# harryjfowen/PointsToWood

Measured on AMD Instinct MI355X. Metric: classified points/sec, higher is better.
Workload: dtype f16x3

## Files before the change

### include/p2w.h

```cpp
#ifndef P2W_H
#define P2W_H

#include <stddef.h>
#include <stdint.h>

#ifdef __cplusplus
extern "C" {
#endif

typedef void* p2w_stream_t;

#define P2W_OK 0
#define P2W_EINVAL (-1)
#define P2W_ENULL (-2)
#define P2W_EALIGN (-3)
#define P2W_EWORKSPACE (-4)
#define P2W_EUNSUPPORTED (-5)

#define P2W_MAX_K 64
#define P2W_MAX_K_WIDE 100
#define P2W_MAX_K_CONV 32

int32_t p2w_version(void);
const char* p2w_strerror(int32_t code);
// ... 36 lines not shown

#define P2W_SEARCH_X_INDEX_IN_W 1
#define P2W_SEARCH_Q_ROW_IN_W 2
#define P2W_SEARCH_BOX 4

int32_t p2w_ball_query(const float* xyzr_x, const int32_t* ptr_x, const float* xyzr_q, const int32_t* qidx,
                       const int32_t* ptr_q, int32_t B, int32_t m_bound, double r, int32_t cap, int32_t* nbr,
                       int32_t* deg, const float* tile_bbox, int32_t flags, p2w_stream_t stream);

int32_t p2w_knn(const float* xyzr_x, const int32_t* ptr_x, const float* xyzr_q, const int32_t* qidx,
                const int32_t* ptr_q, int32_t B, int32_t m_bound, int32_t k, int32_t* nbr, int32_t* deg,
                const float* tile_bbox, int32_t flags, p2w_stream_t stream);

int32_t p2w_knn_grid(const float* xyzr_x, const uint64_t* keys_x, const int32_t* ptr_x, const p2w_grid* grid,
                     const float* xyzr_q, const int32_t* qidx, const int32_t* ptr_q, int32_t B, int32_t m_bound,
                     int32_t k, int32_t* nbr, int32_t* deg, const float* hint, int32_t flags, p2w_stream_t stream);
int32_t p2w_knn_hint2(const float* xyzr_q, const int32_t* rank, const int32_t* ptr_q, int32_t B, int32_t m_bound,
                      const float* xyzr_c, float* hint, p2w_stream_t stream);
int32_t p2w_ball_query_grid(const float* xyzr_x, const uint64_t* keys_x, const int32_t* ptr_x, const p2w_grid* grid,
                            const float* xyzr_q, const int32_t* qidx, const int32_t* ptr_q, int32_t B, int32_t m_bound,
                            double r, int32_t cap, int32_t* nbr, int32_t* deg, int32_t flags, p2w_stream_t stream);
int32_t p2w_voxel_sample_table_prepare(void* ws, size_t ws_bytes, p2w_stream_t stream);
int32_t p2w_voxel_sample_table_prepared(const float* xyzr, const int32_t* ptr, int32_t B, int32_t n_bound, float res,
                                        int32_t* idx_out, int32_t* ptr_out, int32_t* batch_out, int32_t* order_out,
                                        uint64_t* sorted_keys_out, uint64_t* cell_keys_out, p2w_grid* grid_out, int32_t* inv_out,
                                        int32_t* rank_sorted_out, int32_t* cell_start_out, int32_t* cell_start_sorted_out,
                                        int32_t* status_out, int64_t table_cells, void* ws, size_t ws_bytes, p2w_stream_t stream);

int32_t p2w_knn_grid_indexed(const float* xyzr_x, const uint64_t* keys_x, const int32_t* ptr_x, const p2w_grid* grid,
                             const int32_t* cell_start, const float* xyzr_q, const int32_t* qidx, const int32_t* ptr_q, int32_t B,
                             int32_t m_bound, int32_t k, int32_t* nbr, int32_t* deg, const float* hint, int32_t flags,
                             p2w_stream_t stream);
int32_t p2w_ball_query_grid_indexed(const float* xyzr_x, const uint64_t* keys_x, const int32_t* ptr_x, const p2w_grid* grid,
                                    const int32_t* cell_start, const float* xyzr_q, const int32_t* qidx, const int32_t* ptr_q,
                                    int32_t B, int32_t m_bound, double r, int32_t cap, int32_t* nbr, int32_t* deg, int32_t flags,
                                    p2w_stream_t stream);


size_t p2w_morton_order_ws_bytes(int32_t n);
int32_t p2w_morton_order(const float* xyzr, int32_t n, const p2w_grid* grid, int32_t* order_out, void* ws, size_t ws_bytes,
                         p2w_stream_t stream);

#define P2W_CELL_NONFINITE INT64_MAX
int32_t p2w_cells_nd(const float* P, int32_t n, int32_t D, int32_t ld, float size, int64_t* cell_out, void* ws, size_t ws_bytes,
                     p2w_stream_t stream);
size_t p2w_sort_pairs_u64_ws_bytes(int32_t n);
int32_t p2w_sort_pairs_u64(const uint64_t* keys_in, uint64_t* keys_out, const int32_t* vals_in, int32_t* vals_out, int32_t n, void* ws,
                           size_t ws_bytes, p2w_stream_t stream);
size_t p2w_key_runs_ws_bytes(int32_t n);
int32_t p2w_key_runs(const uint64_t* keys_sorted, int32_t n, int32_t min_count, int32_t* starts_out, int32_t* counts_out, int32_t* n_out,
                     void* ws, size_t ws_bytes, p2w_stream_t stream);

size_t p2w_cell_starts_ws_bytes(int64_t n_cells);
int32_t p2w_cell_starts(const uint64_t* keys_sorted, int32_t n, int64_t n_cells, int32_t* table_out, void* ws, size_t ws_bytes,
                        p2w_stream_t stream);

int32_t p2w_knn_refine_f64(const double* cand_sorted, const int32_t* cand_index, const int32_t* cand_pos,
                           const uint64_t* keys_sorted, const int32_t* cell_start, const p2w_grid* grid, double ox, double oy,
                           double oz, const double* q, int32_t m, int32_t nc, int32_t k, int32_t* nbr, int32_t* deg,
                           p2w_stream_t stream);

#define P2W_CLUSTER_LINK 1
#define P2W_CLUSTER_COMPRESS 2
#define P2W_CLUSTER_NUMBER 4
#define P2W_CLUSTER_ALL 7
size_t p2w_euclid_cluster_ws_bytes(int64_t n);
int32_t p2w_euclid_cluster(const double* xyz_sorted, const int32_t* order, const uint64_t* keys_sorted, const int32_t* cell_start,
                           const p2w_grid* grid, int64_t n, double tolerance, int64_t min_size, int64_t max_size, int32_t stages,
                           int64_t* labels_out, int32_t* counts_out, uint64_t* pairs_out, void* ws, size_t ws_bytes,
                           p2w_stream_t stream);

int32_t p2w_knn_wide_f64(const double* xyz_sorted, const int32_t* order, const uint64_t* keys_sorted, const int32_t* cell_start,
                         const p2w_grid* grid, int64_t n, int32_t k, double slack, int32_t* nbr_out, p2w_stream_t stream);

size_t p2w_pathlen_grow_ws_bytes(int64_t n);
int32_t p2w_pathlen_grow(const double* xyz, const int32_t* nbr, int64_t n, int32_t k, int32_t base, int32_t kpairs, double nbrs_threshold,
                         double nbrs_threshold_step, double graph_threshold, int32_t* step_out, int32_t* edges_out, int64_t edge_cap,
                         int64_t* info_out, double* threshold_out, void* ws, size_t ws_bytes, p2w_stream_t stream);

size_t p2w_pathlen_sssp_ws_bytes(int64_t n, int64_t n_edges);
int32_t p2w_pathlen_sssp(const double* xyz, const int32_t* edges, int64_t n_edges, int64_t n, int32_t base, double* dist_out,
                         int32_t* parent_out, int64_t* info_out, void* ws, size_t ws_bytes, p2w_stream_t stream);

int32_t p2w_pathlen_weights(const double* xyz, const int64_t* edges, int64_t n_edges, double* w_out, p2w_stream_t stream);

#define P2W_EVAL_CHUNK 4096
#define P2W_EVAL_MAX_CLASSES 8
size_t p2w_confusion_ws_bytes(int64_t n, int32_t segments, int32_t classes);
int32_t p2w_confusion(const float* truth, const float* pred, const double* weight, const int64_t* seg_ptr, int64_t n, int32_t segments,
                      int32_t classes, int64_t* counts, double* wsum, int64_t* invalid, void* ws, size_t ws_bytes,
                      p2w_stream_t stream);

#define P2W_LOSS_CHUNK 4096
size_t p2w_poly1_focal_ws_bytes(int64_t n);
int32_t p2w_poly1_focal(const float* logits, const float* labels, const float* weight, int64_t weight_n, int64_t n, double epsilon,
                        double gamma, double alpha, double label_smoothing, double eps, float* loss, float* dloss, double* sum,
                        void* ws, size_t ws_bytes, p2w_stream_t stream);

int32_t p2w_vote(const int32_t* nbr, const int32_t* deg, int32_t k, const float* pred, const float* prob, int32_t n,
                 float any_wood, float* label_out, float* pwood_out, p2w_stream_t stream);

int32_t p2w_tile_bbox(const float* xyzr, const int32_t* ptr, int32_t B, int32_t n_bound, float* bbox, p2w_stream_t stream);
int32_t p2w_tile_bbox_count(int32_t B, int32_t n_bound);


int32_t p2w_stem(const float* xyzr, int32_t n, const float* w, const float* b, int32_t C, float* out,
                 p2w_stream_t stream);

typedef struct p2w_epilogue {
    const float* bias;
    const float* sc0;
    const float* sh0;
    const float* sc1;
    const float* sh1;
    const float* residual;
    int32_t ldr;
    int32_t relu0, relu1, relu2, relu_final;
    uint32_t* range;
    const void* interp;
    int32_t interp_rows;
} p2w_epilogue;

#define P2W_RANGE_HI 6.0e4f
#define P2W_RANGE_LO 0.03125f
#define P2W_RANGE_SLOTS 16
#define P2W_RANGE_WORDS (64 * P2W_RANGE_SLOTS)

void p2w_packed_dims(int32_t N, int32_t K, int32_t* N_pad, int32_t* K_pad);

int32_t p2w_gemm(const float* A, int32_t lda, const float* Wp, int32_t M, int32_t N, int32_t K,
                 const p2w_epilogue* epi, float* out, int32_t ldo, p2w_stream_t stream);

int32_t p2w_sa_conv(const float* P, int32_t ldp, const float* xyzr_src, const int32_t* idx, const int32_t* batch_dst,
                    const float* sf, const int32_t* nbr, const int32_t* deg, int32_t kw, int32_t M,
                    const float* w1r4 , const float* W2p, int32_t C1, int32_t C2,
                    const float* b2, const float* bn_s, const float* bn_t, float* out, int32_t ldo,
                    p2w_stream_t stream);

#define P2W_PREC_F16X3 0
#define P2W_PREC_F16 1
#define P2W_PREC_BF16 2
int32_t p2w_packed_dims_h(int32_t prec, int32_t N, int32_t K, int32_t* N_pad, int32_t* K_pad);

#define P2W_GEMM_TILE_128 1
#define P2W_GEMM_TILE_256 2
#define P2W_GEMM_GENERIC_EPI 4
#define P2W_GEMM_ORDER_ROWS 8
#define P2W_GEMM_ORDER_COLS 16
#define P2W_GEMM_RESIDUAL_H 32
#define P2W_GEMM_STREAMK 64
#define P2W_GEMM_NO_STREAMK 128
#define P2W_GEMM_TILE_64 (1 << 24)
#define P2W_GEMM_NO_TILE_64 (1 << 25)
#define P2W_SA_ITEM_256 1
#define P2W_SA_ITEM_128 2
#define P2W_SA_PACK8 4

int32_t p2w_gemm_h2(int32_t prec, const void* A_h, int32_t ldh_a, const void* Wh, float wscale, int32_t M, int32_t N,
                    int32_t K, const p2w_epilogue* epi, float* out_f32, int32_t ldo, void* out_h, int32_t ldh_o,
                    int32_t flags, p2w_stream_t stream);
size_t p2w_gemm_h2_sk_ws_bytes(void);
int32_t p2w_gemm_h2_sk(int32_t prec, const void* A_h, int32_t ldh_a, const void* Wh, float wscale, int32_t M, int32_t N,
                       int32_t K, const p2w_epilogue* epi, float* out_f32, int32_t ldo, void* out_h, int32_t ldh_o,
                       void* ws, size_t ws_bytes, int32_t flags, p2w_stream_t stream);
size_t p2w_gemm_h2_rowdot_ws_bytes(int32_t M, int32_t N);
int32_t p2w_gemm_h2_rowdot(int32_t prec, const void* A_h, int32_t ldh_a, const void* Wh, float wscale, int32_t M, int32_t N,
                           int32_t K, const p2w_epilogue* epi, const float* dot_w, float dot_b, float* out, void* ws,
                           size_t ws_bytes, int32_t flags, p2w_stream_t stream);
size_t p2w_sa_conv_h_ws_bytes(int32_t M, int32_t flags);
int32_t p2w_sa_conv_h(int32_t prec, const float* P, int32_t ldp, int32_t n_src, const float* xyzr_src, const int32_t* idx,
                      const int32_t* batch_dst, const float* sf, const int32_t* nbr, const int32_t* deg, int32_t kw,
                      int32_t M, const float* w1r4, const void* W2h, float wscale, int32_t C1, int32_t C2,
                      const float* b2, const float* bn_s, const float* bn_t, float* out, int32_t ldo, void* out_h,
                      int32_t ldh, void* ws, size_t ws_bytes, int32_t flags, p2w_stream_t stream);
int32_t p2w_sa_conv_h_rows(int32_t prec, const float* P, int32_t ldp, int32_t n_src, const float* xyzr_src, const int32_t* idx,
                           const int32_t* batch_dst, const float* sf, const int32_t* nbr, const int32_t* deg, int32_t kw,
                           int32_t M, const float* w1r4, const void* W2h, float wscale, int32_t C1, int32_t C2,
                           const float* b2, const float* bn_s, const float* bn_t, float* out, int32_t ldo, void* out_h,
                           int32_t ldh, void* ws, size_t ws_bytes, int32_t flags, const int32_t* src_row, uint32_t* range,
                           p2w_stream_t stream);
int32_t p2w_stem_h2(int32_t prec, const float* xyzr, int32_t n, const float* w, const float* b, int32_t C, float* out,
                    void* out_h, int32_t ldh, uint32_t* range, p2w_stream_t stream);
int32_t p2w_stem_h2_indexed(int32_t prec, const float* xyzr, int32_t n, const float* w, const float* b, int32_t C, float* out,
                            void* out_h, int32_t ldh, uint32_t* range, p2w_stream_t stream);
int32_t p2w_interp_concat_h2(int32_t prec, const float* xc, int32_t Fc, const float* xyzr_c, const float* xyzr_f,
                             const int32_t* nbr, const int32_t* deg, int32_t kw, const float* skip, int32_t Fs, int32_t m,
                             void* out_h, int32_t ldh, p2w_stream_t stream);
int32_t p2w_interp_weights(const float* xyzr_c, const float* xyzr_f, const int32_t* nbr, const int32_t* deg, int32_t kw, int32_t m,
                           void* records, p2w_stream_t stream);
int32_t p2w_concat_xyz_h2(int32_t prec, const float* x, int32_t F, const float* xyzr, int32_t m, void* out_h, int32_t ldh,
                          p2w_stream_t stream);

int32_t p2w_interp_concat(const float* xc, int32_t Fc, const float* xyzr_c, const float* xyzr_f, const int32_t* nbr,
                          const int32_t* deg, int32_t kw, const float* skip, int32_t Fs, int32_t m, float* out,
                          int32_t ldo, p2w_stream_t stream);

int32_t p2w_concat_xyz(const float* x, int32_t F, const float* xyzr, int32_t m, float* out, int32_t ldo,
                       p2w_stream_t stream);

int32_t p2w_segment_max(const float* x, int32_t ldx, int32_t F, const int32_t* ptr, int32_t B, float* out,
                        p2w_stream_t stream);

int32_t p2w_rowdot(const float* x, int32_t ldx, int32_t F, const float* w, float b, int32_t m, float* out,
                   p2w_stream_t stream);

int32_t p2w_fill_batch_nbr(const int32_t* batch, int32_t m, int32_t* nbr, int32_t* deg, p2w_stream_t stream);


int32_t p2w_segment_max_arg(const float* x, int32_t ldx, int32_t F, const int32_t* ptr, int32_t B, float* out, int32_t* arg,
                            p2w_stream_t stream);
int32_t p2w_segment_max_bwd(const float* grad_out, int32_t ldg, const int32_t* arg, const int32_t* ptr, int32_t B, int32_t F,
                            float* grad_x, int32_t ldx, int32_t n, p2w_stream_t stream);
size_t p2w_interp_bwd_ws_bytes(int32_t m, int32_t kw, int32_t n_coarse);
int32_t p2w_interp_bwd(const float* grad_out, int32_t ldg, int32_t F, const float* xyzr_c, const float* xyzr_f, const int32_t* nbr,
                       const int32_t* deg, int32_t kw, int32_t m, int32_t n_coarse, float* grad_x, int32_t ldx, void* ws,
                       size_t ws_bytes, p2w_stream_t stream);

int32_t p2w_edge_l1(const float* P, int32_t ldp, const float* rec_src, const float* rec_dst, const int32_t* ptr, const int32_t* src,
                    const float* Wg, int32_t n_src, int32_t M, int32_t E, int32_t C1, float* geo, float* H1, int32_t ldh,
                    p2w_stream_t stream);
#define P2W_EDGE_CHUNK 1024
size_t p2w_edge_l1_bwd_ws_bytes(int32_t E, int32_t n_src, int32_t C1);
int32_t p2w_edge_l1_bwd(const float* gH, int32_t ldg, const float* H1, int32_t ldh, const float* geo, const int32_t* src,
                        const float* Wg, int32_t n_src, int32_t E, int32_t C1, float* gP, int32_t ldgp, float* gR, float* gWg, void* ws,
                        size_t ws_bytes, p2w_stream_t stream);

#define P2W_BN_GROUP 16
size_t p2w_relu_bn_max_ws_bytes(int32_t E, int32_t M, int32_t C2);
int32_t p2w_relu_bn_max(const float* z, int32_t ldz, const int32_t* ptr, const float* gamma, const float* beta, float* running_mean,
                        float* running_var, double momentum, double eps, int32_t E, int32_t M, int32_t C2, float* out, float* ext,
                        int32_t* arg, float* mean, float* invstd, void* ws, size_t ws_bytes, p2w_stream_t stream);
int32_t p2w_relu_bn_max_bwd(const float* g, const float* z, int32_t ldz, const int32_t* ptr, const int32_t* arg, const float* ext,
                            const float* mean, const float* invstd, const float* gamma, int32_t E, int32_t M, int32_t C2, float* dz,
                            int32_t lddz, float* dgamma, float* dbeta, void* ws, size_t ws_bytes, p2w_stream_t stream);

#ifdef __cplusplus
}
#endif
#endif
```

### pointstowood_amd/_lib.py

```python
from __future__ import annotations

import ctypes as C
import os

import torch

_HERE = os.path.dirname(os.path.abspath(__file__))
LIB_PATH = os.path.join(_HERE, "libp2w_gfx950.so")

_vp, _i32, _f32, _sz = C.c_void_p, C.c_int32, C.c_float, C.c_size_t


class Epilogue(C.Structure):
    _fields_ = [("bias", _vp), ("sc0", _vp), ("sh0", _vp), ("sc1", _vp), ("sh1", _vp), ("residual", _vp),
                ("ldr", _i32), ("relu0", _i32), ("relu1", _i32), ("relu2", _i32), ("relu_final", _i32), ("range", _vp),
                ("interp", _vp), ("interp_rows", _i32)]


SEARCH_X_INDEX_IN_W, SEARCH_Q_ROW_IN_W, SEARCH_BOX = 1, 2, 4
PREC_F16X3, PREC_F16, PREC_BF16 = 0, 1, 2
PREC_OF = {"f16x3": PREC_F16X3, "fp16": PREC_F16, "bf16": PREC_BF16}
GEMM_TILE_128, GEMM_TILE_256, GEMM_GENERIC_EPI, GEMM_ORDER_ROWS, GEMM_ORDER_COLS, GEMM_RESIDUAL_H = 1, 2, 4, 8, 16, 32
GEMM_STREAMK, GEMM_NO_STREAMK = 64, 128
SA_ITEM_256, SA_ITEM_128, SA_PACK8 = 1, 2, 4
CLUSTER_LINK, CLUSTER_COMPRESS, CLUSTER_NUMBER, CLUSTER_ALL = 1, 2, 4, 7
MAX_K_WIDE = 100
EVAL_CHUNK, EVAL_MAX_CLASSES = 4096, 8
LOSS_CHUNK = 4096
EDGE_CHUNK = 1024
BN_GROUP = 16

SIGNATURES = {
    "p2w_version": (_i32, []),
    "p2w_strerror": (C.c_char_p, [_i32]),
    "p2w_pack_xyzr": (_i32, [_vp, _i32, _vp, _vp, _i32, _i32, _vp, _vp, _vp]),
    "p2w_voxel_sample_ws_bytes": (_sz, [_i32]),
    "p2w_voxel_sample": (_i32, [_vp, _vp, _i32, _i32, _f32, _vp, _vp, _vp, _vp, _vp, _vp, _vp, _vp, _vp, _vp, _sz, _vp]),
    "p2w_voxel_sample_table_ws_bytes": (_sz, [_i32, C.c_int64]),
    "p2w_voxel_sample_table": (_i32, [_vp, _vp, _i32, _i32, _f32, _vp, _vp, _vp, _vp, _vp, _vp, _vp, _vp, _vp, _vp, _vp, _vp, C.c_int64,
                                      _vp, _sz, _vp]),
    "p2w_voxel_sample_table_prepare": (_i32, [_vp, _sz, _vp]),
    "p2w_voxel_sample_table_prepared": (_i32, [_vp, _vp, _i32, _i32, _f32, _vp, _vp, _vp, _vp, _vp, _vp, _vp, _vp, _vp, _vp, _vp, _vp, C.c_int64,
                                               _vp, _sz, _vp]),
    "p2w_knn_grid_indexed": (_i32, [_vp, _vp, _vp, _vp, _vp, _vp, _vp, _vp, _i32, _i32, _i32, _vp, _vp, _vp, _i32, _vp]),
    "p2w_ball_query_grid_indexed": (_i32, [_vp, _vp, _vp, _vp, _vp, _vp, _vp, _vp, _i32, _i32, C.c_double, _i32, _vp, _vp, _i32, _vp]),
    "p2w_knn_hint2": (_i32, [_vp, _vp, _vp, _i32, _i32, _vp, _vp, _vp]),
    "p2w_knn_grid": (_i32, [_vp, _vp, _vp, _vp, _vp, _vp, _vp, _i32, _i32, _i32, _vp, _vp, _vp, _i32, _vp]),
    "p2w_ball_query_grid": (_i32, [_vp, _vp, _vp, _vp, _vp, _vp, _vp, _i32, _i32, C.c_double, _i32, _vp, _vp, _i32, _vp]),
    "p2w_index_records": (_i32, [_vp, _vp, _vp, _i32, _i32, _vp, _vp]),
    "p2w_voxel_grid": (_i32, [_vp, _vp, _i32, _i32, _f32, _vp, _vp, _sz, _vp]),
    "p2w_consecutive_cluster": (_i32, [_vp, _i32, _vp, _vp, _vp, _vp, _sz, _vp]),
    "p2w_level_gather": (_i32, [_vp, _vp, _vp, _vp, _i32, _i32, _vp, _vp, _vp]),
    "p2w_ball_query": (_i32, [_vp, _vp, _vp, _vp, _vp, _i32, _i32, C.c_double, _i32, _vp, _vp, _vp, _i32, _vp]),
    "p2w_knn": (_i32, [_vp, _vp, _vp, _vp, _vp, _i32, _i32, _i32, _vp, _vp, _vp, _i32, _vp]),
    "p2w_morton_order_ws_bytes": (_sz, [_i32]),
    "p2w_morton_order": (_i32, [_vp, _i32, _vp, _vp, _vp, _sz, _vp]),
    "p2w_cells_nd": (_i32, [_vp, _i32, _i32, _i32, _f32, _vp, _vp, _sz, _vp]),
    "p2w_sort_pairs_u64_ws_bytes": (_sz, [_i32]),
    "p2w_sort_pairs_u64": (_i32, [_vp, _vp, _vp, _vp, _i32, _vp, _sz, _vp]),
    "p2w_key_runs_ws_bytes": (_sz, [_i32]),
    "p2w_key_runs": (_i32, [_vp, _i32, _i32, _vp, _vp, _vp, _vp, _sz, _vp]),
    "p2w_knn_refine_f64": (_i32, [_vp, _vp, _vp, _vp, _vp, _vp, C.c_double, C.c_double, C.c_double, _vp, _i32, _i32, _i32, _vp, _vp, _vp]),
    "p2w_cell_starts_ws_bytes": (_sz, [C.c_int64]),
    "p2w_cell_starts": (_i32, [_vp, _i32, C.c_int64, _vp, _vp, _sz, _vp]),
    "p2w_vote": (_i32, [_vp, _vp, _i32, _vp, _vp, _i32, _f32, _vp, _vp, _vp]),
    "p2w_euclid_cluster_ws_bytes": (_sz, [C.c_int64]),
    "p2w_euclid_cluster": (_i32, [_vp, _vp, _vp, _vp, _vp, C.c_int64, C.c_double, C.c_int64, C.c_int64, _i32, _vp, _vp, _vp, _vp, _sz, _vp]),
    "p2w_knn_wide_f64": (_i32, [_vp, _vp, _vp, _vp, _vp, C.c_int64, _i32, C.c_double, _vp, _vp]),
    "p2w_pathlen_grow_ws_bytes": (_sz, [C.c_int64]),
    "p2w_pathlen_grow": (_i32, [_vp, _vp, C.c_int64, _i32, _i32, _i32, C.c_double, C.c_double, C.c_double, _vp, _vp, C.c_int64, _vp, _vp,
                                _vp, _sz, _vp]),
    "p2w_pathlen_sssp_ws_bytes": (_sz, [C.c_int64, C.c_int64]),
    "p2w_pathlen_sssp": (_i32, [_vp, _vp, C.c_int64, C.c_int64, _i32, _vp, _vp, _vp, _vp, _sz, _vp]),
    "p2w_pathlen_weights": (_i32, [_vp, _vp, C.c_int64, _vp, _vp]),
    "p2w_confusion_ws_bytes": (_sz, [C.c_int64, _i32, _i32]),
    "p2w_confusion": (_i32, [_vp, _vp, _vp, _vp, C.c_int64, _i32, _i32, _vp, _vp, _vp, _vp, _sz, _vp]),
    "p2w_poly1_focal_ws_bytes": (_sz, [C.c_int64]),
    "p2w_poly1_focal": (_i32, [_vp, _vp, _vp, C.c_int64, C.c_int64, C.c_double, C.c_double, C.c_double, C.c_double, C.c_double, _vp, _vp, _vp,
                               _vp, _sz, _vp]),
    "p2w_tile_bbox": (_i32, [_vp, _vp, _i32, _i32, _vp, _vp]),
    "p2w_tile_bbox_count": (_i32, [_i32, _i32]),
    "p2w_stem": (_i32, [_vp, _i32, _vp, _vp, _i32, _vp, _vp]),
    "p2w_packed_dims": (None, [_i32, _i32, C.POINTER(_i32), C.POINTER(_i32)]),
    "p2w_gemm": (_i32, [_vp, _i32, _vp, _i32, _i32, _i32, C.POINTER(Epilogue), _vp, _i32, _vp]),
    "p2w_sa_conv": (_i32, [_vp, _i32, _vp, _vp, _vp, _vp, _vp, _vp, _i32, _i32, _vp, _vp, _i32, _i32, _vp, _vp, _vp,
                           _vp, _i32, _vp]),
    "p2w_packed_dims_h": (_i32, [_i32, _i32, _i32, C.POINTER(_i32), C.POINTER(_i32)]),
    "p2w_gemm_h2": (_i32, [_i32, _vp, _i32, _vp, _f32, _i32, _i32, _i32, C.POINTER(Epilogue), _vp, _i32, _vp, _i32, _i32, _vp]),
    "p2w_gemm_h2_sk_ws_bytes": (_sz, []),
    "p2w_gemm_h2_sk": (_i32, [_i32, _vp, _i32, _vp, _f32, _i32, _i32, _i32, C.POINTER(Epilogue), _vp, _i32, _vp, _i32, _vp, _sz, _i32, _vp]),
    "p2w_gemm_h2_rowdot_ws_bytes": (_sz, [_i32, _i32]),
    "p2w_gemm_h2_rowdot": (_i32, [_i32, _vp, _i32, _vp, _f32, _i32, _i32, _i32, C.POINTER(Epilogue), _vp, _f32, _vp, _vp, _sz, _i32, _vp]),
    "p2w_sa_conv_h_ws_bytes": (_sz, [_i32, _i32]),
    "p2w_sa_conv_h": (_i32, [_i32, _vp, _i32, _i32, _vp, _vp, _vp, _vp, _vp, _vp, _i32, _i32, _vp, _vp, _f32, _i32, _i32, _vp, _vp,
                             _vp, _vp, _i32, _vp, _i32, _vp, _sz, _i32, _vp]),
    "p2w_stem_h2": (_i32, [_i32, _vp, _i32, _vp, _vp, _i32, _vp, _vp, _i32, _vp, _vp]),
    "p2w_stem_h2_indexed": (_i32, [_i32, _vp, _i32, _vp, _vp, _i32, _vp, _vp, _i32, _vp, _vp]),
    "p2w_sa_conv_h_rows": (_i32, [_i32, _vp, _i32, _i32, _vp, _vp, _vp, _vp, _vp, _vp, _i32, _i32, _vp, _vp, _f32, _i32, _i32, _vp, _vp,
                                  _vp, _vp, _i32, _vp, _i32, _vp, _sz, _i32, _vp, _vp, _vp]),
    "p2w_interp_concat_h2": (_i32, [_i32, _vp, _i32, _vp, _vp, _vp, _vp, _i32, _vp, _i32, _i32, _vp, _i32, _vp]),
    "p2w_interp_weights": (_i32, [_vp, _vp, _vp, _vp, _i32, _i32, _vp, _vp]),
    "p2w_concat_xyz_h2": (_i32, [_i32, _vp, _i32, _vp, _i32, _vp, _i32, _vp]),
    "p2w_interp_concat": (_i32, [_vp, _i32, _vp, _vp, _vp, _vp, _i32, _vp, _i32, _i32, _vp, _i32, _vp]),
    "p2w_concat_xyz": (_i32, [_vp, _i32, _vp, _i32, _vp, _i32, _vp]),
    "p2w_segment_max": (_i32, [_vp, _i32, _i32, _vp, _i32, _vp, _vp]),
    "p2w_rowdot": (_i32, [_vp, _i32, _i32, _vp, _f32, _i32, _vp, _vp]),
    "p2w_fill_batch_nbr": (_i32, [_vp, _i32, _vp, _vp, _vp]),
    "p2w_segment_max_arg": (_i32, [_vp, _i32, _i32, _vp, _i32, _vp, _vp, _vp]),
    "p2w_segment_max_bwd": (_i32, [_vp, _i32, _vp, _vp, _i32, _i32, _vp, _i32, _i32, _vp]),
    "p2w_interp_bwd_ws_bytes": (_sz, [_i32, _i32, _i32]),
    "p2w_interp_bwd": (_i32, [_vp, _i32, _i32, _vp, _vp, _vp, _vp, _i32, _i32, _i32, _vp, _i32, _vp, _sz, _vp]),
    "p2w_edge_l1": (_i32, [_vp, _i32, _vp, _vp, _vp, _vp, _vp, _i32, _i32, _i32, _i32, _vp, _vp, _i32, _vp]),
    "p2w_edge_l1_bwd_ws_bytes": (_sz, [_i32, _i32, _i32]),
    "p2w_edge_l1_bwd": (_i32, [_vp, _i32, _vp, _i32, _vp, _vp, _vp, _i32, _i32, _i32, _vp, _i32, _vp, _vp, _vp, _sz, _vp]),
    "p2w_relu_bn_max_ws_bytes": (_sz, [_i32, _i32, _i32]),
    "p2w_relu_bn_max": (_i32, [_vp, _i32, _vp, _vp, _vp, _vp, _vp, C.c_double, C.c_double, _i32, _i32, _i32, _vp, _vp, _vp, _vp, _vp, _vp, _sz,
                               _vp]),
    "p2w_relu_bn_max_bwd": (_i32, [_vp, _vp, _i32, _vp, _vp, _vp, _vp, _vp, _vp, _i32, _i32, _i32, _vp, _i32, _vp, _vp, _vp, _sz, _vp]),
}

_lib = None


def lib():
    global _lib
    if _lib is None:
        from . import build as _build
        if _build._stale():
            try:
                _build.build()
            except Exception as e:
                raise RuntimeError(
                    f"{LIB_PATH} is missing or stale and could not be rebuilt ({e}). The HIP extension is the "
                    "only compute path (no CPU fallback). Build it with `python -m pointstowood_amd.build`.") from e
        h = C.CDLL(LIB_PATH)
        for name, (res, args) in SIGNATURES.items():
            fn = getattr(h, name)
            fn.restype, fn.argtypes = res, args
        _lib = h
    return _lib


def check(code: int, what: str = "") -> None:
    if code != 0:
        msg = lib().p2w_strerror(code).decode()
        raise RuntimeError(f"{what or 'p2w'} failed: {msg} (code {code})")


def ptr(t):
    return None if t is None else t.data_ptr()


_raw_stream = getattr(torch._C, "_cuda_getCurrentRawStream", None)
_raw_device = getattr(torch._C, "_cuda_getDevice", None)


def stream():
    if _raw_stream is not None and _raw_device is not None:
        return _raw_stream(_raw_device())
    return torch.cuda.current_stream().cuda_stream


def stage_timer(on: bool):
    events = []

    def mark():
        if on:
            events.append(torch.cuda.Event(enable_timing=True))
            events[-1].record()

    def ms():
        events[-1].synchronize()
        return [a.elapsed_time(b) for a, b in zip(events[:-1], events[1:])]
    return mark, ms


def require_cuda(*tensors):
    for t in tensors:
        if t is not None and not t.is_cuda:
            raise RuntimeError("pointstowood_amd operators need tensors on an MI355X (cuda) device; "
                               "there is no CPU fallback")


def aligned16(t):
    return t.clone() if t.data_ptr() % 16 else t


def packed_dims(n: int, k: int, prec: int | None = None):
    a, b = _i32(), _i32()
    if prec is None:
        lib().p2w_packed_dims(n, k, C.byref(a), C.byref(b))
    else:
        check(lib().p2w_packed_dims_h(prec, n, k, C.byref(a), C.byref(b)), "p2w_packed_dims_h")
    return a.value, b.value
```

### pointstowood_amd/csrc/p2w_feat.hip

```cpp
#include "p2w_hgemm.h"

constexpr int G_BM = 128, G_BN = 128, G_BK = 32, G_LD = 36;

extern "C" void p2w_packed_dims(int32_t N, int32_t K, int32_t* N_pad, int32_t* K_pad) {
    if (N_pad) *N_pad = (N + 255) / 256 * 256;
    if (K_pad) *K_pad = (K + G_BK - 1) / G_BK * G_BK;
}
extern "C" int32_t p2w_packed_dims_h(int32_t prec, int32_t N, int32_t K, int32_t* N_pad, int32_t* K_pad) {
    if (prec < P2W_PREC_F16X3 || prec > P2W_PREC_BF16) return P2W_EINVAL;
    const int ka = prec == P2W_PREC_F16X3 ? 32 : 64;
    if (N_pad) *N_pad = (N + 255) / 256 * 256;
    if (K_pad) *K_pad = (K + ka - 1) / ka * ka;
    return P2W_OK;
}

__device__ __forceinline__ void mma_slab(const float* __restrict__ As, const float* __restrict__ Bs, int wr, int wc, int lane,
                                         f32x16 (&acc)[2][2]) {
    const int r = lane & 31, h = lane >> 5;
#pragma unroll
    for (int kk = 0; kk < G_BK; kk += 8) {
        const float4 a0 = *reinterpret_cast<const float4*>(&As[(wr * 64 + r) * G_LD + kk + 4 * h]);
        const float4 a1 = *reinterpret_cast<const float4*>(&As[(wr * 64 + 32 + r) * G_LD + kk + 4 * h]);
        const float4 b0 = *reinterpret_cast<const float4*>(&Bs[(wc * 64 + r) * G_LD + kk + 4 * h]);
        const float4 b1 = *reinterpret_cast<const float4*>(&Bs[(wc * 64 + 32 + r) * G_LD + kk + 4 * h]);
// ... 129 lines not shown
    const int h = lane >> 5;
#pragma unroll
    for (int i = 0; i < 2; ++i) {
        const int tgt = t0 + wr * 2 + i;
        if (tgt >= M) continue;
        const int d = min(deg[tgt], kw);
#pragma unroll
        for (int j = 0; j < 2; ++j) {
            const int col = n0 + wc * 64 + j * 32 + (lane & 31);
            const bool cv = col < C2;
            const float bias = cv ? b2[col] : 0.f, s = cv ? bn_s[col] : 0.f, t = cv ? bn_t[col] : 0.f;
            float vmax = -INFINITY;
#pragma unroll
            for (int r = 0; r < 16; ++r) {
                const int slot = (r & 3) + 8 * (r >> 2) + 4 * h;
                const float v = fmaf(fmaxf(fmaf(acc[i][j][r], wscale, bias), 0.f), s, t);
                if (slot < d) vmax = fmaxf(vmax, v);
            }
            vmax = fmaxf(vmax, __shfl_xor(vmax, 32));
            if (d == 0) vmax = 0.f;
            if (cv && h == 0) out[(size_t)tgt * ldo + col] = vmax;
        }
    }
}

__device__ __forceinline__ void sa_row_geometry(int tid, int t0, int M, int kw, const float4* __restrict__ xyzr,
                                                const int* __restrict__ idx, const int* __restrict__ batch_dst,
                                                const float* __restrict__ sf, const int* __restrict__ nbr,
                                                const int* __restrict__ deg, int* m_j, float (*m_g)[4]) {
    if (tid < G_BM) {
        const int tgt = t0 + (tid >> 5), slot = tid & 31;
        int j = 0;
        float rx = 0.f, ry = 0.f, rz = 0.f, rf = 0.f, nrm = 0.f;
        if (tgt < M) {
            const int d = deg[tgt];
            const float s = sf[batch_dst[tgt]];
            const float4 pi = xyzr[idx[tgt]];
            const bool valid = slot < d && slot < kw;
            j = nbr[(size_t)tgt * kw + (valid ? slot : 0)];
            if (j < 0) j = idx[tgt];
            const float4 pj = xyzr[j];
            if (valid) {
                rx = pj.x / s - pi.x / s; ry = pj.y / s - pi.y / s; rz = pj.z / s - pi.z / s;
                nrm = sqrtf(((rx * rx) + (ry * ry)) + (rz * rz));
                rf = pj.w;
            }
        }
        float dmax = nrm;
#pragma unroll
        for (int off = 16; off >= 1; off >>= 1) dmax = fmaxf(dmax, __shfl_xor(dmax, off));
        const float den = dmax + 1e-8f;
        m_j[tid] = j;
        m_g[tid][0] = rx / den; m_g[tid][1] = ry / den; m_g[tid][2] = rz / den; m_g[tid][3] = rf;
    }
}

__device__ __forceinline__ void sa_load_h1(const float* __restrict__ P, int ldp, const float* __restrict__ w1r4, int C1,
                                           int C1pad, int k, const int (&rj)[4], const float4 (&rg)[4], float4 (&ra)[4]) {
    if (k < C1) {
        const float4 wx = *reinterpret_cast<const float4*>(&w1r4[0 * C1pad + k]);
        const float4 wy = *reinterpret_cast<const float4*>(&w1r4[1 * C1pad + k]);
        const float4 wz = *reinterpret_cast<const float4*>(&w1r4[2 * C1pad + k]);
        const float4 wf = *reinterpret_cast<const float4*>(&w1r4[3 * C1pad + k]);
#pragma unroll
        for (int i = 0; i < 4; ++i) {
            const float4 p = *reinterpret_cast<const float4*>(&P[(size_t)rj[i] * ldp + k]);
            const float4 g = rg[i];
            float4 v;
            v.x = fmaxf(fmaf(g.w, wf.x, fmaf(g.z, wz.x, fmaf(g.y, wy.x, fmaf(g.x, wx.x, p.x)))), 0.f);
            v.y = fmaxf(fmaf(g.w, wf.y, fmaf(g.z, wz.y, fmaf(g.y, wy.y, fmaf(g.x, wx.y, p.y)))), 0.f);
            v.z = fmaxf(fmaf(g.w, wf.z, fmaf(g.z, wz.z, fmaf(g.y, wy.z, fmaf(g.x, wx.z, p.z)))), 0.f);
            v.w = fmaxf(fmaf(g.w, wf.w, fmaf(g.z, wz.w, fmaf(g.y, wy.w, fmaf(g.x, wx.w, p.w)))), 0.f);
            ra[i] = v;
        }
    } else {
#pragma unroll
        for (int i = 0; i < 4; ++i) ra[i] = make_float4(0.f, 0.f, 0.f, 0.f);
    }
}

__global__ __launch_bounds__(256) void sa_conv_kernel(const float* __restrict__ P, int ldp, const float4* __restrict__ xyzr,
                                                      const int* __restrict__ idx, const int* __restrict__ batch_dst,
                                                      const float* __restrict__ sf, const int* __restrict__ nbr,
                                                      const int* __restrict__ deg, int kw, int M,
                                                      const float* __restrict__ w1r4, int C1, int C1pad,
                                                      const float* __restrict__ W2p, int C2, int nMt, int nNt,
                                                      const float* __restrict__ b2, const float* __restrict__ bn_s,
                                                      const float* __restrict__ bn_t, float* __restrict__ out, int ldo) {
    __shared__ __attribute__((aligned(16))) float As[G_BM * G_LD];
    __shared__ __attribute__((aligned(16))) float Bs[G_BN * G_LD];
    __shared__ int m_j[G_BM];
    __shared__ float m_g[G_BM][4];
    int mt, nt;
    if (!tile_coords(nMt, nNt, &mt, &nt)) return;
    const int t0 = mt * 4, n0 = nt * G_BN;
    const int tid = threadIdx.x, lane = tid & 63, wave = tid >> 6, wr = wave >> 1, wc = wave & 1;
    const int lrow = tid >> 3, lkq = tid & 7;

    sa_row_geometry(tid, t0, M, kw, xyzr, idx, batch_dst, sf, nbr, deg, m_j, m_g);
    __syncthreads();
    int rj[4];
    float4 rg[4];
#pragma unroll
    for (int i = 0; i < 4; ++i) {
        rj[i] = m_j[lrow + 32 * i];
        rg[i] = *reinterpret_cast<const float4*>(&m_g[lrow + 32 * i][0]);
    }

    f32x16 acc[2][2];
#pragma unroll
    for (int i = 0; i < 2; ++i)
#pragma unroll
        for (int j = 0; j < 2; ++j)
#pragma unroll
            for (int r = 0; r < 16; ++r) acc[i][j][r] = 0.f;

    float4 ra[4], rb[4];
    sa_load_h1(P, ldp, w1r4, C1, C1pad, 4 * lkq, rj, rg, ra);
    load_w_tile(W2p, C1pad, n0, 0, lrow, lkq, rb);
    for (int k0 = 0; k0 < C1pad; k0 += G_BK) {
        __syncthreads();
        store_tile(As, lrow, lkq, ra);
        store_tile(Bs, lrow, lkq, rb);
        __syncthreads();
        if (k0 + G_BK < C1pad) {
            sa_load_h1(P, ldp, w1r4, C1, C1pad, k0 + G_BK + 4 * lkq, rj, rg, ra);
            load_w_tile(W2p, C1pad, n0, k0 + G_BK, lrow, lkq, rb);
        }
        mma_slab(As, Bs, wr, wc, lane, acc);
    }

    sa_epilogue(acc, 1.0f, t0, n0, wr, wc, lane, M, kw, deg, C2, b2, bn_s, bn_t, out, ldo);
}

extern "C" int32_t p2w_sa_conv(const float* P, int32_t ldp, const float* xyzr_src, const int32_t* idx, const int32_t* batch_dst,
                               const float* sf, const int32_t* nbr, const int32_t* deg, int32_t kw, int32_t M,
                               const float* w1r4, const float* W2p, int32_t C1, int32_t C2, const float* b2,
                               const float* bn_s, const float* bn_t, float* out, int32_t ldo, p2w_stream_t stream) {
    if (M == 0) return P2W_OK;
    P2W_CHECK_PTR(P); P2W_CHECK_PTR(xyzr_src); P2W_CHECK_PTR(idx); P2W_CHECK_PTR(batch_dst); P2W_CHECK_PTR(sf);
    P2W_CHECK_PTR(nbr); P2W_CHECK_PTR(deg); P2W_CHECK_PTR(w1r4); P2W_CHECK_PTR(W2p); P2W_CHECK_PTR(b2);
    P2W_CHECK_PTR(bn_s); P2W_CHECK_PTR(bn_t); P2W_CHECK_PTR(out);
    P2W_CHECK_ALIGN16(P); P2W_CHECK_ALIGN16(xyzr_src); P2W_CHECK_ALIGN16(w1r4); P2W_CHECK_ALIGN16(W2p);
    if (M < 0 || kw <= 0 || kw > 32 || C1 <= 0 || C2 <= 0 || (C1 & 3) || (ldp & 3) || ldp < C1 || ldo < C2) return P2W_EINVAL;
    int C2pad, C1pad;
    p2w_packed_dims(C2, C1, &C2pad, &C1pad);
    const int nMt = p2w_cdiv(M, 4), nNt = p2w_cdiv(C2, G_BN);
    sa_conv_kernel<<<tile_grid(nMt, nNt), 256, 0, p2w_s(stream)>>>(
        P, ldp, reinterpret_cast<const float4*>(xyzr_src), idx, batch_dst, sf, nbr, deg, kw, M, w1r4, C1, C1pad, W2p, C2,
        nMt, nNt, b2, bn_s, bn_t, out, ldo);
    return P2W_LAUNCH_STATUS();
}

static int32_t gemm_h2_checked(int32_t prec, const void* A_h, int32_t ldh_a, const void* Wh, float wscale, int32_t M, int32_t N,
                               int32_t K, const p2w_epilogue* epi, float* out_f32, int32_t ldo, void* out_h, int32_t ldh_o,
                               void* ws, size_t ws_bytes, int32_t flags, p2w_stream_t stream) {
    if (prec < P2W_PREC_F16X3 || prec > P2W_PREC_BF16) return P2W_EINVAL;
    if (ws) P2W_CHECK_ALIGN16(ws);
    if ((flags & P2W_GEMM_STREAMK) && (flags & P2W_GEMM_NO_STREAMK)) return P2W_EINVAL;
    if (M == 0) return P2W_OK;
    P2W_CHECK_PTR(A_h); P2W_CHECK_PTR(Wh);
    if (!out_f32 && !out_h) return P2W_ENULL;
    P2W_CHECK_ALIGN16(A_h); P2W_CHECK_ALIGN16(Wh);
    if (out_h) P2W_CHECK_ALIGN16(out_h);
    if (M < 0 || N <= 0 || K <= 0 || ldh_a < K || !(wscale > 0.f)) return P2W_EINVAL;
    if (out_f32 && ldo < N) return P2W_EINVAL;
    if (out_h && ldh_o < N) return P2W_EINVAL;
    if ((flags & P2W_GEMM_TILE_128) && (flags & P2W_GEMM_TILE_256)) return P2W_EINVAL;
    EpiArgs ep = {};
    if (epi) {
        if ((epi->sc0 && !epi->sh0) || (epi->sc1 && !epi->sh1)) return P2W_ENULL;
        if (epi->residual && epi->ldr < N) return P2W_EINVAL;
        ep = {epi->bias, epi->sc0, epi->sh0, epi->sc1, epi->sh1, epi->residual,
              epi->ldr, epi->relu0, epi->relu1, epi->relu2, epi->relu_final, nullptr, epi->range, nullptr};
        if (epi->interp) {
            if (!epi->residual) return P2W_ENULL;
            if (flags & P2W_GEMM_RESIDUAL_H) return P2W_EUNSUPPORTED;
            if (reinterpret_cast<uintptr_t>(epi->interp) & 15u) return P2W_EALIGN;
            if (epi->interp_rows <= 0 || (size_t)epi->interp_rows * (size_t)epi->ldr >= ((size_t)1 << 31)) return P2W_EINVAL;
            ep.imeta = static_cast<const int4*>(epi->interp);
        }
        if ((flags & P2W_GEMM_RESIDUAL_H) && epi->residual) {
            if ((epi->ldr & 7) || (reinterpret_cast<uintptr_t>(epi->residual) & 15u)) return P2W_EALIGN;
            ep.res_h = reinterpret_cast<const _Float16*>(epi->residual);
            ep.residual = nullptr;
        }
    }
    const _Float16* Ah = static_cast<const _Float16*>(A_h);
    const _Float16* Wp = static_cast<const _Float16*>(Wh);
    if (prec == P2W_PREC_F16X3)
        return launch_gemm_h<0>(Ah, ldh_a, Wp, wscale, M, N, K, ep, out_f32, ldo, static_cast<_Float16*>(out_h), ldh_o, flags,
                                p2w_s(stream), nullptr, nullptr, 0, static_cast<float*>(ws), ws_bytes);
    return p2w_gemm_h1_impl(prec, Ah, ldh_a, Wp, wscale, M, N, K, ep, out_f32, ldo, static_cast<_Float16*>(out_h), ldh_o, flags,
                            p2w_s(stream), nullptr, nullptr, 0, static_cast<float*>(ws), ws_bytes);
}
extern "C" int32_t p2w_gemm_h2(int32_t prec, const void* A_h, int32_t ldh_a, const void* Wh, float wscale, int32_t M, int32_t N,
                               int32_t K, const p2w_epilogue* epi, float* out_f32, int32_t ldo, void* out_h, int32_t ldh_o,
                               int32_t flags, p2w_stream_t stream) {
    return gemm_h2_checked(prec, A_h, ldh_a, Wh, wscale, M, N, K, epi, out_f32, ldo, out_h, ldh_o, nullptr, 0, flags, stream);
}
extern "C" size_t p2w_gemm_h2_sk_ws_bytes(void) { return (size_t)2 * p2w_cu_count() * 128 * 128 * sizeof(float); }
extern "C" int32_t p2w_gemm_h2_sk(int32_t prec, const void* A_h, int32_t ldh_a, const void* Wh, float wscale, int32_t M, int32_t N,
                                  int32_t K, const p2w_epilogue* epi, float* out_f32, int32_t ldo, void* out_h, int32_t ldh_o,
                                  void* ws, size_t ws_bytes, int32_t flags, p2w_stream_t stream) {
    if (!ws && ws_bytes) return P2W_ENULL;
    return gemm_h2_checked(prec, A_h, ldh_a, Wh, wscale, M, N, K, epi, out_f32, ldo, out_h, ldh_o, ws, ws_bytes, flags, stream);
}

__global__ __launch_bounds__(256) void rowdot_finish_kernel(const float* __restrict__ part, int ldpart, int nslots, float b, int M,
                                                            float* __restrict__ out) {
    const int i = blockIdx.x * 256 + threadIdx.x;
    if (i >= M) return;
    float acc = 0.f;
    for (int s = 0; s < nslots; ++s) acc = acc + part[(size_t)s * ldpart + i];
    out[i] = acc + b;
}
static inline int rowdot_ldpart(int M) { return (M + 255) / 256 * 256; }
extern "C" size_t p2w_gemm_h2_rowdot_ws_bytes(int32_t M, int32_t N) {
    if (M < 0 || N <= 0) return 0;
    return (size_t)((N + 63) / 64) * rowdot_ldpart(M) * sizeof(float);
}
extern "C" int32_t p2w_gemm_h2_rowdot(int32_t prec, const void* A_h, int32_t ldh_a, const void* Wh, float wscale, int32_t M, int32_t N,
                                      int32_t K, const p2w_epilogue* epi, const float* dot_w, float dot_b, float* out, void* ws,
                                      size_t ws_bytes, int32_t flags, p2w_stream_t stream) {
    if (prec < P2W_PREC_F16X3 || prec > P2W_PREC_BF16) return P2W_EINVAL;
    if (M == 0) return P2W_OK;
    P2W_CHECK_PTR(A_h); P2W_CHECK_PTR(Wh); P2W_CHECK_PTR(dot_w); P2W_CHECK_PTR(out); P2W_CHECK_PTR(ws);
    P2W_CHECK_ALIGN16(A_h); P2W_CHECK_ALIGN16(Wh); P2W_CHECK_ALIGN16(ws);
    if (M < 0 || N <= 0 || K <= 0 || ldh_a < K || !(wscale > 0.f)) return P2W_EINVAL;
    if ((flags & P2W_GEMM_TILE_128) && (flags & P2W_GEMM_TILE_256)) return P2W_EINVAL;
    if (ws_bytes < p2w_gemm_h2_rowdot_ws_bytes(M, N)) return P2W_EWORKSPACE;
    EpiArgs ep = {};
    if (epi) {
        if ((epi->sc0 && !epi->sh0) || (epi->sc1 && !epi->sh1)) return P2W_ENULL;
        if (epi->residual || epi->interp) return P2W_EUNSUPPORTED;
        ep = {epi->bias, epi->sc0, epi->sh0, epi->sc1, epi->sh1, nullptr, 0, epi->relu0, epi->relu1, epi->relu2, epi->relu_final, nullptr, epi->range, nullptr};
    }
    const _Float16* Ah = static_cast<const _Float16*>(A_h);
    const _Float16* Wp = static_cast<const _Float16*>(Wh);
    float* part = static_cast<float*>(ws);
    const int ldpart = rowdot_ldpart(M);
    const int32_t rc = prec == P2W_PREC_F16X3
        ? launch_gemm_h<0>(Ah, ldh_a, Wp, wscale, M, N, K, ep, nullptr, 0, nullptr, 0, flags, p2w_s(stream), dot_w, part, ldpart)
        : p2w_gemm_h1_impl(prec, Ah, ldh_a, Wp, wscale, M, N, K, ep, nullptr, 0, nullptr, 0, flags, p2w_s(stream), dot_w, part, ldpart);
    if (rc != P2W_OK) return rc;
    rowdot_finish_kernel<<<p2w_cdiv(M, 256), 256, 0, p2w_s(stream)>>>(part, ldpart, (N + 63) / 64, dot_b, M, out);
    return P2W_LAUNCH_STATUS();
}

__global__ __launch_bounds__(256) void sa_edge_meta_kernel(const float4* __restrict__ xyzr, const int* __restrict__ idx,
                                                           const int* __restrict__ batch_dst, const float* __restrict__ sf,
                                                           const int* __restrict__ nbr, const int* __restrict__ deg, int kw,
                                                           int M, int n_src, int ldp4, int G, const int* __restrict__ list,
                                                           const int* __restrict__ n_list_dev, const int* __restrict__ src_row,
                                                           int* __restrict__ meta_j, float4* __restrict__ meta_g, int* __restrict__ desc,
                                                           float4* __restrict__ zero_row) {
    const long g = (long)blockIdx.x * 256 + threadIdx.x;
    if (zero_row && g < ldp4) zero_row[g] = make_float4(0.f, 0.f, 0.f, 0.f);
    const int n_groups = list ? *n_list_dev : M;
    const int gpt = 32 / G;
    const long n_tiles = ((long)n_groups + gpt - 1) / gpt;
    if (g >= n_tiles * 32) return;
    const int gi = (int)(g / G), slot = (int)(g % G);
    const int tgt = gi < n_groups ? (list ? list[gi] : gi) : -1;
    int j = 0, d = 0;
    float rx = 0.f, ry = 0.f, rz = 0.f, rf = 0.f, nrm = 0.f;
    bool valid = false;
    if (tgt >= 0) {
        d = min(deg[tgt], kw);
        const int self = idx[tgt];
        const float s = sf[batch_dst[tgt]];
        const float4 pi = xyzr[self];
        valid = slot < d;
        j = valid ? nbr[(size_t)tgt * kw + slot] : self;
        if (j < 0) j = self;
        const float4 pj = xyzr[j];
        if (valid) {
            rx = pj.x / s - pi.x / s; ry = pj.y / s - pi.y / s; rz = pj.z / s - pi.z / s;
            nrm = sqrtf(((rx * rx) + (ry * ry)) + (rz * rz));
            rf = pj.w;
        }
    }
    float dmax = nrm;
    for (int off = G >> 1; off >= 1; off >>= 1) dmax = fmaxf(dmax, __shfl_xor(dmax, off));
    const float den = dmax + 1e-8f;
    meta_j[g] = (valid ? (src_row ? src_row[j] : j) : n_src) * ldp4;
    meta_g[g] = make_float4(rx / den, ry / den, rz / den, rf);
    if (slot == 0) desc[gi] = tgt >= 0 ? ((tgt << 6) | d) : -1;
}

__global__ __launch_bounds__(SA_PART_BLOCK) void sa_part_count_kernel(const int* __restrict__ deg, int kw, int M, int* __restrict__ blk_small) {
    const int t = blockIdx.x * SA_PART_BLOCK + threadIdx.x;
    const bool small = t < M && min(deg[t], kw) <= 8;
    const int c = __syncthreads_count(small);
    if (threadIdx.x == 0) blk_small[blockIdx.x] = c;
}
__global__ __launch_bounds__(1024) void sa_part_scan_kernel(int* __restrict__ blk_small, int nblk, int M, int* __restrict__ counts) {
    __shared__ int part[1024];
    const int per = (nblk + 1023) / 1024, b0 = threadIdx.x * per, b1 = min(b0 + per, nblk);
    int sum = 0;
    for (int b = b0; b < b1; ++b) sum += blk_small[b];
    part[threadIdx.x] = sum;
    __syncthreads();
    for (int off = 1; off < 1024; off <<= 1) {
        const int v = threadIdx.x >= off ? part[threadIdx.x - off] : 0;
        __syncthreads();
        part[threadIdx.x] += v;
        __syncthreads();
    }
    int run = part[threadIdx.x] - sum;
    for (int b = b0; b < b1; ++b) { const int c = blk_small[b]; blk_small[b] = run; run += c; }
    if (threadIdx.x == 1023) {
        const int ns = part[1023], nl = M - ns;
        counts[0] = ns; counts[1] = nl; counts[2] = (ns + 3) / 4; counts[3] = nl;
    }
}
__global__ __launch_bounds__(SA_PART_BLOCK) void sa_part_scatter_kernel(const int* __restrict__ deg, int kw, int M, const int* __restrict__ blk_small,
                                                                     int* __restrict__ list_small, int* __restrict__ list_large) {
    __shared__ int wsum[SA_PART_BLOCK / 64];
    const int t = blockIdx.x * SA_PART_BLOCK + threadIdx.x, lane = threadIdx.x & 63, wave = threadIdx.x >> 6;
    const bool in = t < M, small = in && min(deg[t], kw) <= 8;
    const unsigned long long bal = __ballot(small);
    const int r_in_wave = __popcll(bal & ((1ull << lane) - 1ull));
    if (lane == 0) wsum[wave] = __popcll(bal);
    __syncthreads();
    int before = 0;
    for (int w = 0; w < wave; ++w) before += wsum[w];
    const int off_s = blk_small[blockIdx.x];
    const int rank_s = before + r_in_wave;
    if (small) list_small[off_s + rank_s] = t;
    else if (in) list_large[(blockIdx.x * SA_PART_BLOCK - off_s) + (threadIdx.x - rank_s)] = t;
}

extern "C" size_t p2w_sa_conv_h_ws_bytes(int32_t M, int32_t flags) { return sa_conv_ws_bytes(M < 0 ? 0 : M, flags); }

extern "C" int32_t p2w_sa_conv_h_rows(int32_t prec, const float* P, int32_t ldp, int32_t n_src, const float* xyzr_src, const int32_t* idx,
                                 const int32_t* batch_dst, const float* sf, const int32_t* nbr, const int32_t* deg,
                                 int32_t kw, int32_t M, const float* w1r4, const void* W2h, float wscale, int32_t C1,
                                 int32_t C2, const float* b2, const float* bn_s, const float* bn_t, float* out,
                                 int32_t ldo, void* out_h, int32_t ldh, void* ws, size_t ws_bytes, int32_t flags,
                                 const int32_t* src_row, uint32_t* range, p2w_stream_t stream) {
    if (prec < P2W_PREC_F16X3 || prec > P2W_PREC_BF16) return P2W_EINVAL;
    if (M == 0) return P2W_OK;
    P2W_CHECK_PTR(P); P2W_CHECK_PTR(xyzr_src); P2W_CHECK_PTR(idx); P2W_CHECK_PTR(batch_dst); P2W_CHECK_PTR(sf);
    P2W_CHECK_PTR(nbr); P2W_CHECK_PTR(deg); P2W_CHECK_PTR(w1r4); P2W_CHECK_PTR(W2h); P2W_CHECK_PTR(b2);
    P2W_CHECK_PTR(bn_s); P2W_CHECK_PTR(bn_t);
    if (!out && !out_h) return P2W_ENULL;
    P2W_CHECK_ALIGN16(P); P2W_CHECK_ALIGN16(xyzr_src); P2W_CHECK_ALIGN16(w1r4); P2W_CHECK_ALIGN16(W2h);
    if (M < 0 || n_src < 0 || kw <= 0 || kw > 32 || C1 <= 0 || C2 <= 0 || (C1 & 3) || (ldp & 3) || ldp < C1 || (out && ldo < C2) ||
        (out_h && (ldh < C2 || (ldh & 7))) || !(wscale > 0.f))
        return P2W_EINVAL;
    const _Float16* W2 = static_cast<const _Float16*>(W2h);
    if (prec == P2W_PREC_F16X3)
        return launch_sa_conv_h<0>(P, ldp, n_src, xyzr_src, idx, batch_dst, sf, nbr, deg, kw, M, w1r4, W2, wscale, C1, C2, b2, bn_s, bn_t,
                                   out, ldo, static_cast<_Float16*>(out_h), ldh, ws, ws_bytes, flags, p2w_s(stream), src_row, range);
    return p2w_sa_conv_h1_impl(prec, P, ldp, n_src, xyzr_src, idx, batch_dst, sf, nbr, deg, kw, M, w1r4, W2, wscale, C1, C2, b2, bn_s,
                               bn_t, out, ldo, static_cast<_Float16*>(out_h), ldh, ws, ws_bytes, flags, p2w_s(stream), src_row, range);
}

// ... 355 lines not shown
```

### pointstowood_amd/csrc/p2w_feat_h1.hip

```cpp
#include "p2w_hgemm.h"

int32_t p2w_gemm_h1_impl(int32_t prec, const _Float16* Ah, int32_t ldh_a, const _Float16* Wp, float wscale, int32_t M, int32_t N,
                         int32_t K, const EpiArgs& ep, float* out_f32, int32_t ldo, _Float16* out_h2, int32_t ldh_o,
                         int32_t flags, hipStream_t stream, const float* dotw, float* part, int32_t ldpart, float* skws,
                         size_t skws_bytes) {
    if (prec == P2W_PREC_F16)
        return launch_gemm_h<1>(Ah, ldh_a, Wp, wscale, M, N, K, ep, out_f32, ldo, out_h2, ldh_o, flags, stream, dotw, part, ldpart, skws, skws_bytes);
    return launch_gemm_h<2>(Ah, ldh_a, Wp, wscale, M, N, K, ep, out_f32, ldo, out_h2, ldh_o, flags, stream, dotw, part, ldpart, skws, skws_bytes);
}

int32_t p2w_sa_conv_h1_impl(int32_t prec, const float* P, int32_t ldp, int32_t n_src, const float* xyzr_src, const int32_t* idx,
                            const int32_t* batch_dst, const float* sf, const int32_t* nbr, const int32_t* deg, int32_t kw,
                            int32_t M, const float* w1r4, const _Float16* W2h, float wscale, int32_t C1, int32_t C2,
                            const float* b2, const float* bn_s, const float* bn_t, float* out, int32_t ldo, _Float16* out_h2,
                            int32_t ldh, void* ws, size_t ws_bytes, int32_t flags, hipStream_t stream, const int32_t* src_row,
                            unsigned* range) {
    if (prec == P2W_PREC_F16)
        return launch_sa_conv_h<1>(P, ldp, n_src, xyzr_src, idx, batch_dst, sf, nbr, deg, kw, M, w1r4, W2h, wscale, C1, C2, b2, bn_s, bn_t,
                                   out, ldo, out_h2, ldh, ws, ws_bytes, flags, stream, src_row, range);
    return launch_sa_conv_h<2>(P, ldp, n_src, xyzr_src, idx, batch_dst, sf, nbr, deg, kw, M, w1r4, W2h, wscale, C1, C2, b2, bn_s, bn_t,
                               out, ldo, out_h2, ldh, ws, ws_bytes, flags, stream, src_row, range);
}
```

### pointstowood_amd/csrc/p2w_hgemm.h

```cpp
#pragma once
#include "p2w_common.h"
#include <type_traits>

typedef float f32x16 __attribute__((ext_vector_type(16)));
typedef _Float16 h8 __attribute__((ext_vector_type(8)));
typedef __bf16 bf8 __attribute__((ext_vector_type(8)));
typedef __fp16 hpair __attribute__((ext_vector_type(2)));
typedef _Float16 hpairn __attribute__((ext_vector_type(2)));
typedef __bf16 bpair __attribute__((ext_vector_type(2)));
typedef float fpair __attribute__((ext_vector_type(2)));
typedef __attribute__((address_space(3))) void* lds_vp;
typedef const __attribute__((address_space(1))) void* glb_vp;

constexpr int H_BK = 32;
constexpr int SA_EPI_COLS = 1024;

template <int PREC> struct HCfg {
    static constexpr int planes = PREC == 0 ? 2 : 1;
    static constexpr int kslab = PREC == 0 ? 32 : 64;
    static constexpr int kalign = PREC == 0 ? 32 : 64;
};

template <int PREC>
__device__ __forceinline__ f32x16 h_mfma(h8 a, h8 b, f32x16 c) {
// ... 224 lines not shown
        if constexpr (RI_OK) {
            if (RI) {
                int4 m0[RI_D];
#pragma unroll
                for (int d = 0; d < RI_D; ++d) m0[d] = ep.imeta[row_of(d)];
                if (RI_D < NSTEP) m_nxt = ep.imeta[row_of(RI_D)];
#pragma unroll
                for (int d = 0; d < RI_D; ++d) load_zrows(d, m0[d]);
            }
        }
        if (RES && !RI) load_res(rcur, 0);
    }
    float dot4[4] = {0.f, 0.f, 0.f, 0.f};
    unsigned long long r_over = 0ull, r_seen = 0ull;
    float m4 = 0.f;
#pragma unroll
    for (int st = 0; st < NSTEP; ++st) {
        const int it = st >> 2, reg = st & 3;
        const int row = row_of(st);
        if constexpr (!GEN) {
            if constexpr (RI_OK) {
                if (RI) {
#pragma unroll
                    for (int jq = 0; jq < JQ; ++jq)
                        rcur[jq] = fpair{fmaf(a1r[st % RI_D], z1r[st % RI_D][jq][0], a0r[st % RI_D] * z0r[st % RI_D][jq][0]),
                                         fmaf(a1r[st % RI_D], z1r[st % RI_D][jq][1], a0r[st % RI_D] * z0r[st % RI_D][jq][1])};
                    if (st + RI_D < NSTEP) {
                        load_zrows(st % RI_D, m_nxt);
                        if (st + RI_D + 1 < NSTEP) m_nxt = ep.imeta[row_of(st + RI_D + 1)];
                    }
                }
            }
            if (RES && !RI && st + 1 < NSTEP) load_res(rnxt, st + 1);
            __builtin_amdgcn_sched_barrier(0);
            float* fp = OF ? o.f32 + ((unsigned)row * (unsigned)o.ldo + (unsigned)cb) : nullptr;
            _Float16* hp = nullptr;
            if (OH) {
                if constexpr (PREC == 0) hp = o.h2 + ((unsigned)row * (unsigned)(2 * o.ldh) + (unsigned)(64 * (cb >> 5) + (cb & 31)));
                else hp = o.h2 + ((unsigned)row * (unsigned)o.ldh + (unsigned)cb);
            }
            float dsum = 0.f;
#pragma unroll
            for (int jq = 0; jq < JQ; ++jq) {
                const float va = value(acc[it][2 * jq][reg], bias[jq][0], s0[jq][0], t0[jq][0], s1[jq][0], t1[jq][0], rcur[jq][0]);
                const float vb = value(acc[it][2 * jq + 1][reg], bias[jq][1], s0[jq][1], t0[jq][1], s1[jq][1], t1[jq][1], rcur[jq][1]);
                m4 = nan_max(nan_max(m4, fabsf(va)), fabsf(vb));
                if (DOT) dsum = fmaf(vb, dw[jq][1], fmaf(va, dw[jq][0], dsum));
                if (OF) *reinterpret_cast<fpair*>(fp + 32 * jq) = fpair{va, vb};
                if (OH) {
                    if constexpr (PREC == 0) {
                        unsigned hw, lw;
                        split_pair(va, vb, hw, lw);
                        *reinterpret_cast<unsigned*>(hp + 64 * jq) = hw;
                        *reinterpret_cast<unsigned*>(hp + 64 * jq + 32) = lw;
                    } else {
                        *reinterpret_cast<unsigned*>(hp + 32 * jq) = pack_pair<PREC>(va, vb);
                    }
                }
            }
            if (reg == 3) {
                r_over |= __ballot(!(m4 <= P2W_RANGE_HI));
                r_seen |= __ballot(m4 > P2W_RANGE_LO);
                m4 = 0.f;
            }
            if (DOT) {
                dot4[reg] = row16_sum(dsum);
                if (reg == 3 && c16 == 0)
                    *reinterpret_cast<float4*>(o.part + ((unsigned)(col0 >> 6) * (unsigned)o.ldpart + (unsigned)(row - 3))) =
                        make_float4(dot4[0], dot4[1], dot4[2], dot4[3]);
            }
            if (RES && !RI) {
#pragma unroll
                for (int jq = 0; jq < JQ; ++jq) rcur[jq] = rnxt[jq];
            }
        } else {
            float dsum = 0.f;
            if (row < M) {
                int4 mt = make_int4(0, 0, 0, 0);
                if constexpr (RI_OK) {
                    if (RI) mt = ep.imeta[row];
                }
#pragma unroll
                for (int jq = 0; jq < JQ; ++jq) {
                    const int c = cb + 32 * jq;
                    float v[2];
#pragma unroll
                    for (int e = 0; e < 2; ++e) {
                        const bool cv = c + e < N;
                        float res = 0.f;
                        if (RI && cv) res = fmaf(__int_as_float(mt.w), ep.residual[(size_t)mt.y * ep.ldr + c + e], __int_as_float(mt.z) * ep.residual[(size_t)mt.x * ep.ldr + c + e]);
                        else if (RES && cv) res = RH ? h_load2<PREC>(ep.res_h, (unsigned)ep.ldr, (unsigned)row, (unsigned)c)[e] : ep.residual[(size_t)row * ep.ldr + c + e];
                        v[e] = value(acc[it][2 * jq + e][reg], bias[jq][e], s0[jq][e], t0[jq][e], s1[jq][e], t1[jq][e], res);
                        if (!cv) v[e] = 0.f;
                        if (OF && cv) o.f32[(size_t)row * o.ldo + c + e] = v[e];
                    }
                    {
                        const float m2 = nan_max(fabsf(v[0]), fabsf(v[1]));
                        r_over |= __ballot(!(m2 <= P2W_RANGE_HI));
                        r_seen |= __ballot(m2 > P2W_RANGE_LO);
                    }
                    if (DOT) dsum = fmaf(v[1], dw[jq][1], fmaf(v[0], dw[jq][0], dsum));
                    if (OH && c < o.hcols) h_store2<PREC>(o.h2, o.ldh, row, c, v[0], v[1]);
                }
            }
            if (DOT) {
                dsum = row16_sum(dsum);
                if (row < M && c16 == 0 && col0 < N) o.part[(size_t)(col0 >> 6) * o.ldpart + row] = dsum;
            }
        }
    }
    if (ep.range) range_commit(ep.range, r_over != 0ull, seen_report && r_seen != 0ull, lane);
}

constexpr int p2w_vmcnt_imm(int n) { return (n & 15) | (7 << 4) | (15 << 8) | ((n >> 4) << 14); }

template <int PREC, int RT16, int CT16, bool WAIT_OLDER = false, bool DOTK = false>
__device__ __forceinline__ void gemm_epilogue_dispatch16(const f32x4 (&acc)[RT16][CT16], const EpiArgs& ep, float wscale, int row0,
                                                         int col0, int lane, int M, int N, const OutArgs& o, int ef,
                                                         bool seen_report = true) {
    const bool full = (row0 + 16 * RT16 <= M) && (col0 + 16 * CT16 <= N) && ef != 0;
    if (full) {
        if constexpr (DOTK) {
            if (ef == 513) {
                gemm_epilogue_16<PREC, RT16, CT16, 513, true>(acc, ep, wscale, row0, col0, lane, M, N, o, seen_report);
                if constexpr (WAIT_OLDER) __builtin_amdgcn_s_waitcnt(p2w_vmcnt_imm(RT16 < 63 ? RT16 : 63));
                return;
            }
        } else
        switch (ef) {
#define P2W_EPI_CASE(E) case E: { \
            gemm_epilogue_16<PREC, RT16, CT16, E>(acc, ep, wscale, row0, col0, lane, M, N, o, seen_report); \
            constexpr int n_st = RT16 * 4 * (CT16 / 2) * (((E) & 128 ? 1 : 0) + ((E) & 256 ? (PREC == 0 ? 2 : 1) : 0)) ; \
            if constexpr (WAIT_OLDER) __builtin_amdgcn_s_waitcnt(p2w_vmcnt_imm(n_st < 63 ? n_st : 63)); \
            return; }
            P2W_EPI_CASE(128) P2W_EPI_CASE(257) P2W_EPI_CASE(263) P2W_EPI_CASE(287) P2W_EPI_CASE(224)
            P2W_EPI_CASE(131) P2W_EPI_CASE(259) P2W_EPI_CASE(387) P2W_EPI_CASE(129)
            P2W_EPI_CASE(480) P2W_EPI_CASE(1376) P2W_EPI_CASE(1504)
#undef P2W_EPI_CASE
            case 2400:
                if constexpr (!DOTK && RT16 <= 4) {
                    gemm_epilogue_16<PREC, RT16, CT16, 2400>(acc, ep, wscale, row0, col0, lane, M, N, o, seen_report);
                    constexpr int n_st = RT16 * 4 * (CT16 / 2) * (PREC == 0 ? 2 : 1);
                    if constexpr (WAIT_OLDER) __builtin_amdgcn_s_waitcnt(p2w_vmcnt_imm(n_st < 63 ? n_st : 63));
                    return;
                }
                break;
            default: break;
        }
    }
    gemm_epilogue_16<PREC, RT16, CT16, -1, DOTK>(acc, ep, wscale, row0, col0, lane, M, N, o, seen_report);
    if constexpr (WAIT_OLDER) __builtin_amdgcn_s_waitcnt(p2w_vmcnt_imm(0));
}

template <int PREC, int WR, int WC, int RT, int CT, bool DOTK, bool SK>
__device__ __forceinline__ void gemm_hp_body(const _Float16* __restrict__ A, int ldh_a, const _Float16* __restrict__ Wh, float wscale,
                                             int M, int N, int Kpad, int nMt, int nNt, int nvb, const EpiArgs& ep, const OutArgs& o,
                                             int ef, int tmode, int sk_S, float* __restrict__ skws) {
    constexpr int KS = HCfg<PREC>::kslab;
    constexpr int BM = 32 * RT * WR, BN = 32 * CT * WC, NW = WR * WC;
    constexpr int A_CH = 8 * BM, STAGE_CH = A_CH + 8 * BN;
    constexpr bool HALF = NW == 8;
    constexpr int NWI = HALF ? NW / 2 : NW;
    constexpr int NI = STAGE_CH / 64 / NWI;
    static_assert(STAGE_CH % (64 * NWI) == 0, "stage must split evenly over the issuing waves");
    __shared__ __attribute__((aligned(16))) char S[2 * STAGE_CH * 16];
    const int tid = threadIdx.x, lane = tid & 63;
    const int wave = __builtin_amdgcn_readfirstlane(tid >> 6), wr = wave / WC, wc = wave % WC;
    const size_t a_pitch = (size_t)HCfg<PREC>::planes * ldh_a, w_pitch = (size_t)HCfg<PREC>::planes * Kpad;
    auto next_tile = [&](int& L, int& mt_, int& nt_) {
        while (L < nvb) {
            if (tile_coords_at(L, nMt, nNt, &mt_, &nt_, tmode)) return true;
            L += gridDim.x;
        }
        return false;
    };
    const int nslab = Kpad / KS;
    int L = blockIdx.x, mt, nt;
    int sk_s0 = 0, sk_s1 = 0, sk_piece = 0;
    if constexpr (SK) {
        const int P = nvb * sk_S, per_xcd = (P + 7) >> 3;
        const int w = blockIdx.x >> 3;
        sk_piece = (blockIdx.x & 7) * per_xcd + w;
        if (w >= per_xcd || sk_piece >= P) return;
        const int j = sk_piece / nvb, r = sk_piece - j * nvb;
        sk_s0 = (int)((long long)j * nslab / sk_S);
        sk_s1 = (int)((long long)(j + 1) * nslab / sk_S);
        if (sk_s0 >= sk_s1) return;
        mt = r / nNt; nt = r - mt * nNt;
    } else if (!next_tile(L, mt, nt)) {
        return;
    }

    const _Float16* src[NI];
    auto setup_src = [&](int mt_, int nt_) {
#pragma unroll
        for (int i = 0; i < NI; ++i) {
            const int g = (wave % NWI) + NWI * i;
            const int row = 8 * g + (lane >> 3);
            const int c = (lane & 7) ^ ((row >> 1) & 7);
            if (g < BM / 8) src[i] = A + (size_t)min(mt_ * BM + row, M - 1) * a_pitch + 8 * c;
            else src[i] = Wh + (size_t)(nt_ * BN + w_stage_row16(row - BM)) * w_pitch + 8 * c;
        }
    };
    const unsigned lds_base = (unsigned)(uintptr_t)(lds_vp)S;
    auto issue_piece = [&](int i, int stage, int k0) {
        const int g = (wave % NWI) + NWI * i;
        const unsigned dst = lds_base + (unsigned)(stage * STAGE_CH + g * 64) * 16u;
        asm volatile("s_mov_b32 m0, %1\n\ts_nop 0\n\tglobal_load_lds_dwordx4 %0, off"
                     :: "v"(src[i] + k0), "s"(dst) : "m0", "memory");
    };
    const bool issuer = wave < NWI;
    constexpr int RT16 = 2 * RT, CT16 = 2 * CT;
    const int r16 = lane & 15, kg = lane >> 4;
    int offA[RT16], offB[CT16];
#pragma unroll
    for (int t = 0; t < RT16; ++t) {
        const int ra = wr * 32 * RT + 16 * t + r16;
        offA[t] = (ra * 8 + (kg ^ ((ra >> 1) & 7))) * 16;
    }
#pragma unroll
    for (int t = 0; t < CT16; ++t) {
        const int rb = BM + wc * 32 * CT + 16 * t + r16;
        offB[t] = (rb * 8 + (kg ^ ((rb >> 1) & 7))) * 16;
    }
    setup_src(mt, nt);
    if (issuer) {
#pragma unroll
        for (int i = 0; i < NI; ++i) issue_piece(i, 0, SK ? sk_s0 * 64 : 0);
    }
    int gs = 0;
    bool landed = false;
    f32x4 acc[RT16][CT16];
    h8 ah[RT16 / 2], al[RT16 / 2], bh[CT16], bl[CT16];
    auto slab = [&](int s, auto last_c, int mtn, int ntn) {
        constexpr bool LAST = decltype(last_c)::value;
        asm volatile("" ::: "memory");
        if (landed) __builtin_amdgcn_s_waitcnt(0xC07F);
        else __builtin_amdgcn_s_waitcnt(0x0070);
        landed = false;
        __builtin_amdgcn_s_barrier();
        asm volatile("" ::: "memory");
        if constexpr (LAST) setup_src(mtn, ntn);
        constexpr int HR = RT16 / 2;
        constexpr int NG = 2 * HR * CT16;
        constexpr int GAP = (NG / (2 * NI)) > 0 ? NG / (2 * NI) : 1;
        const int k_next = LAST ? 0 : (s + 1) * 64;
        if constexpr (HALF) {
            if (issuer) {
#pragma unroll
                for (int i = 0; i < NI; ++i) issue_piece(i, (gs + 1) & 1, k_next);
            }
        }
        const char* st = S + (size_t)(gs & 1) * STAGE_CH * 16;
#pragma unroll
        for (int t = 0; t < CT16; ++t) {
            bh[t] = *reinterpret_cast<const h8*>(st + offB[t]);
            bl[t] = *reinterpret_cast<const h8*>(st + (offB[t] ^ 64));
        }
#pragma unroll
        for (int hh = 0; hh < 2; ++hh) {
#pragma unroll
            for (int t = 0; t < HR; ++t) {
                ah[t] = *reinterpret_cast<const h8*>(st + offA[hh * HR + t]);
                al[t] = *reinterpret_cast<const h8*>(st + (offA[hh * HR + t] ^ 64));
            }
#pragma unroll
            for (int i = 0; i < HR; ++i)
#pragma unroll
                for (int j = 0; j < CT16; ++j) {
                    f32x4& c = acc[hh * HR + i][j];
                    if constexpr (PREC == 0) {
                        c = h_mfma16<PREC>(al[i], bh[j], c);
                        c = h_mfma16<PREC>(ah[i], bl[j], c);
                        c = h_mfma16<PREC>(ah[i], bh[j], c);
                    } else {
                        c = h_mfma16<PREC>(ah[i], bh[j], c);
                        c = h_mfma16<PREC>(al[i], bl[j], c);
                    }
                    if constexpr (!HALF) {
                        const int g = (hh * HR + i) * CT16 + j;
                        if ((g % GAP) == GAP - 1 && g / GAP < NI) {
                            issue_piece(g / GAP, (gs + 1) & 1, k_next);
                            __builtin_amdgcn_sched_barrier(0);
                        }
                    }
                }
        }
        ++gs;
    };
    if constexpr (SK) {
#pragma unroll
        for (int i = 0; i < RT16; ++i)
#pragma unroll
            for (int j = 0; j < CT16; ++j) acc[i][j] = f32x4{0.f, 0.f, 0.f, 0.f};
        for (int s = sk_s0; s + 1 < sk_s1; ++s) slab(s, std::false_type{}, 0, 0);
        slab(sk_s1 - 1, std::true_type{}, mt, nt);
        f32x4* dst = reinterpret_cast<f32x4*>(skws) + (size_t)sk_piece * (size_t)(BM * BN / 4) + tid;
#pragma unroll
        for (int i = 0; i < RT16; ++i)
#pragma unroll
            for (int j = 0; j < CT16; ++j) dst[(i * CT16 + j) * (64 * NW)] = acc[i][j];
    } else {
    while (true) {
        int Ln = L + gridDim.x, mtn = mt, ntn = nt;
        const bool more = next_tile(Ln, mtn, ntn);
        if (!more) { mtn = mt; ntn = nt; }
#pragma unroll
        for (int i = 0; i < RT16; ++i)
#pragma unroll
            for (int j = 0; j < CT16; ++j) acc[i][j] = f32x4{0.f, 0.f, 0.f, 0.f};
        for (int s = 0; s + 1 < nslab; ++s) slab(s, std::false_type{}, 0, 0);
        slab(nslab - 1, std::true_type{}, mtn, ntn);
        gemm_epilogue_dispatch16<PREC, RT16, CT16, true, DOTK>(acc, ep, wscale, mt * BM + wr * 32 * RT, nt * BN + wc * 32 * CT, lane, M, N, o, ef,
                                                               gs == nslab && wave == 0);
        landed = true;
        if (!more) break;
        L = Ln; mt = mtn; nt = ntn;
    }
    }
    asm volatile("s_waitcnt vmcnt(0)" ::: "memory");
}

template <int PREC, int WR, int WC, int RT, int CT, bool DOTK = false>
__global__ __launch_bounds__(64 * WR * WC, 2) void gemm_hp_kernel(const _Float16* __restrict__ A, int ldh_a,
                                                               const _Float16* __restrict__ Wh, float wscale, int M, int N,
                                                               int Kpad, int nMt, int nNt, int nvb, EpiArgs ep, OutArgs o, int ef,
                                                               int tmode) {
    gemm_hp_body<PREC, WR, WC, RT, CT, DOTK, false>(A, ldh_a, Wh, wscale, M, N, Kpad, nMt, nNt, nvb, ep, o, ef, tmode, 0, nullptr);
}

template <int PREC>
__global__ __launch_bounds__(256, 3) void gemm_hp64_kernel(const _Float16* __restrict__ A, int ldh_a, const _Float16* __restrict__ Wh,
                                                        float wscale, int M, int N, int Kpad, int nMt, int nNt, int nvb, EpiArgs ep,
                                                        OutArgs o, int ef, int tmode) {
    gemm_hp_body<PREC, 2, 2, 1, 2, false, false>(A, ldh_a, Wh, wscale, M, N, Kpad, nMt, nNt, nvb, ep, o, ef, tmode, 0, nullptr);
}

template <int PREC, int WR, int WC, int RT, int CT>
__global__ __launch_bounds__(64 * WR * WC, 2) void gemm_hp_sk_kernel(const _Float16* __restrict__ A, int ldh_a,
                                                                  const _Float16* __restrict__ Wh, int M, int Kpad, int nNt,
                                                                  int tiles, int S, float* __restrict__ skws) {
    const EpiArgs ep = {};
    const OutArgs o = {};
    gemm_hp_body<PREC, WR, WC, RT, CT, false, true>(A, ldh_a, Wh, 1.f, M, 0, Kpad, 0, nNt, tiles, ep, o, 0, 0, S, skws);
}

template <int PREC, int WR, int WC, int RT, int CT>
__global__ __launch_bounds__(64 * WR * WC) void gemm_hp_skfix_kernel(const float* __restrict__ skws, int tiles, int S, int nslab, int nNt,
                                                                      float wscale, int M, int N, EpiArgs ep, OutArgs o, int ef) {
    constexpr int BM = 32 * RT * WR, BN = 32 * CT * WC, NW = WR * WC, RT16 = 2 * RT, CT16 = 2 * CT;
    const int tid = threadIdx.x, lane = tid & 63;
    const int wave = __builtin_amdgcn_readfirstlane(tid >> 6), wr = wave / WC, wc = wave % WC;
    const int r = blockIdx.x / RT16, i = blockIdx.x - r * RT16;
    f32x4 acc[1][CT16];
#pragma unroll
    for (int j = 0; j < CT16; ++j) acc[0][j] = f32x4{0.f, 0.f, 0.f, 0.f};
    for (int p = 0; p < S; ++p) {
        if ((int)((long long)p * nslab / S) >= (int)((long long)(p + 1) * nslab / S)) continue;
        const f32x4* src = reinterpret_cast<const f32x4*>(skws) + (size_t)(p * tiles + r) * (size_t)(BM * BN / 4) + tid;
#pragma unroll
        for (int jj = 0; jj < CT16; ++jj) acc[0][jj] += src[(i * CT16 + jj) * (64 * NW)];
    }
    const int mt = r / nNt, nt = r - mt * nNt;
    gemm_epilogue_dispatch16<PREC, 1, CT16, false, false>(acc, ep, wscale, mt * BM + wr * 32 * RT + 16 * i, nt * BN + wc * 32 * CT, lane, M, N, o, ef);
}

template <int PREC>
static int32_t launch_gemm_h(const _Float16* Ah, int32_t ldh_a, const _Float16* Wp, float wscale, int32_t M, int32_t N, int32_t K,
                             const EpiArgs& ep, float* out_f32, int32_t ldo, _Float16* out_h2, int32_t ldh_o, int32_t flags,
                             hipStream_t stream, const float* dotw = nullptr, float* part = nullptr, int32_t ldpart = 0,
                             float* skws = nullptr, size_t skws_bytes = 0, int sk_S = 0) {
    constexpr int KA = HCfg<PREC>::kalign;
    const int Npad = (N + 255) / 256 * 256, Kpad = (K + KA - 1) / KA * KA;
    if (ep.imeta) flags = (flags & ~P2W_GEMM_TILE_256) | P2W_GEMM_TILE_128;
    if ((ldh_a % KA) != 0 || ldh_a < Kpad) return P2W_EINVAL;
    if (out_h2 && (ldh_o & 7)) return P2W_EINVAL;
    const int hcols = ldh_o < (N + KA - 1) / KA * KA ? ldh_o : (N + KA - 1) / KA * KA;
    OutArgs o = {out_f32, ldo, out_h2, ldh_o, hcols, dotw, part, ldpart};
    const int n_cu = p2w_cu_count();
    auto pick_big = [&](int rows) {
        const long tiles256 = (long)p2w_cdiv(rows, 256) * (Npad / 256);
        const long rounds = (tiles256 + n_cu - 1) / n_cu;
        const bool fills = tiles256 * 100 >= rounds * n_cu * 78;
        bool b = N >= 256 && (N % 256) == 0 && tiles256 * 4 >= 3 * n_cu && fills;
        if (flags & P2W_GEMM_TILE_256) b = true;
        if (flags & P2W_GEMM_TILE_128) b = false;
        return b;
    };
    const bool big = pick_big(M);
    bool t64 = false;
    if (!dotw && sk_S == 0 && !ep.imeta && !(flags & (P2W_GEMM_TILE_128 | P2W_GEMM_TILE_256 | P2W_GEMM_NO_TILE_64))) {
        if (flags & P2W_GEMM_TILE_64) t64 = true;
        else if (K <= 1024 && N <= 192) t64 = true;
        else if (K <= 1024 && !big) {
            const long nNt1 = p2w_cdiv(N, 128), T128 = (long)p2w_cdiv(M, 128) * nNt1, T64 = (long)p2w_cdiv(M, 64) * nNt1;
            const long S128 = 2L * n_cu, S64 = 3L * n_cu;
            const double w128 = (double)((T128 + S128 - 1) / S128 * S128) / (double)T128, w64 = (double)((T64 + S64 - 1) / S64 * S64) / (double)T64;
            t64 = T128 <= 2 * S128 && w128 >= 1.3 * w64;
        }
    }
    if (sk_S == 0 && skws && !dotw && !t64 && !(flags & P2W_GEMM_NO_STREAMK)) {
        const int nslab = Kpad / HCfg<PREC>::kslab;
        const double f = PREC == 0 ? 1.0 : 0.7, ts1 = 0.9 * f, ts2 = 1.65 * f, tsb = 2.25 * f;
        auto t_small = [&](long tiles) { return tiles > n_cu ? ts2 : ts1; };
        auto t_big = [&](long tiles) { return tiles >= n_cu ? tsb : (0.75 * f + (tsb - 0.75 * f) * (double)tiles / n_cu); };
        auto one_launch = [&](bool b, int rows) {
            const long T = b ? (long)p2w_cdiv(rows, 256) * (Npad / 256) : (long)p2w_cdiv(rows, 128) * p2w_cdiv(N, 128);
            const long G = b ? n_cu : 2 * n_cu, qq = T / G, R = T % G;
            return (double)nslab * ((double)qq * (b ? tsb : ts2) + (R ? (b ? t_big(R) : t_small(R)) : 0.0));
        };
        const bool big_ok = N >= 256 && (N % 256) == 0;
        double best_cost = one_launch(big, M);
        int best_mode = 0, best_rows_full = 0, best_S = 0;
        bool best_big = big, sk_big = big, tail_big = false;
        double sk_cost = 1e30;
        int sk_rows_full = 0, sk_S_best = 0;
        const size_t piece_b = (size_t)128 * 128 * 4;
        for (int cand = 0; cand < 2; ++cand) {
            const bool b = cand == 0;
            if (b && !(N >= 256 && (N % 256) == 0)) continue;
            if ((flags & P2W_GEMM_TILE_256) && !b) continue;
            if ((flags & P2W_GEMM_TILE_128) && b) continue;
            const int BMm = b ? 256 : 128, G_m = n_cu * (b ? 1 : 2);
            const int nNt_m = b ? Npad / 256 : p2w_cdiv(N, 128), nMt_m = p2w_cdiv(M, BMm);
            const long T = (long)nMt_m * nNt_m, q = T / G_m;
            const int mt_full = (int)((q * G_m) / nNt_m);
            if ((long)mt_full * nNt_m >= T) continue;
            if (q == 0 && b != big) continue;
            const int rows_full = mt_full * BMm, m_t = M - rows_full;
            const double main_t = (double)q * nslab * (b ? tsb : ts2) + (q > 0 ? 4.0 : 0.0);
            const long T_t = (long)p2w_cdiv(m_t, 128) * p2w_cdiv(N, 128);
            if (q > 0) {
                for (int tb = 0; tb < 2; ++tb) {
                    if (tb == 1 && (!big_ok || (flags & P2W_GEMM_TILE_128))) continue;
                    if (tb == 0 && (flags & P2W_GEMM_TILE_256)) continue;
                    const double c = main_t + one_launch(tb == 1, m_t);
                    if (c < 0.95 * best_cost) { best_cost = c; best_mode = 1; best_rows_full = rows_full; best_big = b; best_S = 0; tail_big = tb == 1; }
                }
            }
            for (int S = 2; S <= nslab && T_t * S <= 2 * n_cu; ++S) {
                if ((size_t)(T_t * S) * piece_b > skws_bytes) break;
                const double c = main_t + (double)((nslab + S - 1) / S) * 1.0 * f + 18.0 + (double)(T_t * S) * piece_b * 2.0 / 8.0e6;
                if (c < sk_cost) { sk_cost = c; sk_rows_full = rows_full; sk_big = b; sk_S_best = S; }
            }
        }
        if (sk_S_best > 0 && (sk_cost < 0.9 * best_cost || (flags & P2W_GEMM_STREAMK))) {
            best_mode = 2; best_rows_full = sk_rows_full; best_big = sk_big; best_S = sk_S_best;
        }
        if (best_mode != 0) {
            constexpr int PL = HCfg<PREC>::planes;
            const int fl = (flags & ~(P2W_GEMM_STREAMK | P2W_GEMM_TILE_128 | P2W_GEMM_TILE_256)) | P2W_GEMM_NO_STREAMK;
            const int rows_full = best_rows_full, m_t = M - rows_full;
            if (rows_full > 0) {
                const int32_t rc = launch_gemm_h<PREC>(Ah, ldh_a, Wp, wscale, rows_full, N, K, ep, out_f32, ldo, out_h2, ldh_o,
                                                       fl | (best_big ? P2W_GEMM_TILE_256 : P2W_GEMM_TILE_128), stream);
                if (rc != P2W_OK) return rc;
            }
            const size_t r0 = (size_t)rows_full;
            EpiArgs ept = ep;
            if (ept.imeta) ept.imeta += r0;
            else if (ept.residual) ept.residual += r0 * ep.ldr;
            if (ept.res_h) ept.res_h += r0 * PL * ep.ldr;
            return launch_gemm_h<PREC>(Ah + r0 * PL * ldh_a, ldh_a, Wp, wscale, m_t, N, K, ept, out_f32 ? out_f32 + r0 * ldo : nullptr, ldo,
                                       out_h2 ? out_h2 + r0 * PL * ldh_o : nullptr, ldh_o,
                                       best_mode == 2 ? fl : (fl | (tail_big ? P2W_GEMM_TILE_256 : P2W_GEMM_TILE_128)), stream, nullptr, nullptr, 0,
                                       best_mode == 2 ? skws : nullptr, skws_bytes, best_mode == 2 ? best_S : 0);
        }
    }
    int ef = (ep.relu0 ? 1 : 0) | (ep.sc0 ? 2 : 0) | (ep.relu1 ? 4 : 0) | (ep.sc1 ? 8 : 0) | (ep.relu2 ? 16 : 0) |
             ((ep.residual || ep.res_h) ? 32 : 0) | (ep.relu_final ? 64 : 0) | (out_f32 ? 128 : 0) | (out_h2 ? 256 : 0) | (dotw ? 512 : 0) |
             (ep.res_h ? 1024 : 0) | (ep.imeta ? 2048 : 0);
    const size_t lim = (size_t)1 << 31;
    if ((size_t)M * (size_t)(ldo > 2 * ldh_o ? ldo : 2 * ldh_o) >= lim || ((ep.residual || ep.res_h) && !ep.imeta && (size_t)M * (size_t)ep.ldr * (ep.res_h ? 2 : 1) >= lim) ||
        (N & 1) || (flags & P2W_GEMM_GENERIC_EPI))
        ef = 0;
    auto odd8 = [](const void* q) { return (reinterpret_cast<uintptr_t>(q) & 7) != 0; };
    if ((out_f32 && ((ldo & 1) || odd8(out_f32))) || (ep.residual && ((ep.ldr & 1) || odd8(ep.residual))) || odd8(ep.bias) ||
        (ep.res_h && ((ep.ldr & 7) || (reinterpret_cast<uintptr_t>(ep.res_h) & 15))) ||
        odd8(ep.sc0) || odd8(ep.sh0) || odd8(ep.sc1) || odd8(ep.sh1) || odd8(dotw) || (part && ((ldpart & 3) || (reinterpret_cast<uintptr_t>(part) & 15))))
        ef = 0;
    const size_t w_bytes = (size_t)N * Kpad * 2 * HCfg<PREC>::planes, a_bytes = (size_t)M * Kpad * 2 * HCfg<PREC>::planes;
    auto pick_mode = [&](int nNtx, int nMtx, int per_cu) {
        const bool ok = nNtx >= 8 || (nNtx > 0 && 8 % nNtx == 0);
        if (!ok) return 0;
        if (flags & P2W_GEMM_ORDER_ROWS) return 0;
        if (flags & P2W_GEMM_ORDER_COLS) return 1;
        const size_t l2_keep = (size_t)3 * 1024 * 1024;
        const int wpx = n_cu / 8 * per_cu;
        const int R = wpx / nNtx > 0 ? wpx / nNtx : 1;
        const int rows_px = p2w_cdiv(nMtx, 8), xcds = nMtx < 8 ? nMtx : 8;
        const size_t t_rows = a_bytes * (size_t)p2w_cdiv(nNtx, wpx) + w_bytes * xcds * (w_bytes <= l2_keep ? 1 : p2w_cdiv(rows_px, R));
        size_t t_cols;
        if (nNtx >= 8) {
            const int cpx = p2w_cdiv(nNtx, 8), Rc = wpx / cpx > 0 ? wpx / cpx : 1;
            t_cols = a_bytes * 8 + w_bytes * (w_bytes / 8 <= l2_keep ? 1 : p2w_cdiv(nMtx, Rc));
        } else {
            t_cols = a_bytes * nNtx + w_bytes * 8 / nNtx;
        }
        return t_cols * 10 < t_rows * 9 ? 1 : 0;
    };
    auto pgrid = [&](int nvb, int per_cu) {
        const int cap = n_cu * per_cu;
        int g = nvb < cap ? nvb : cap;
        if (g >= 8) g &= ~7;
        return g;
    };
    if (sk_S > 0) {
        const int nslab = Kpad / HCfg<PREC>::kslab, nNt1 = p2w_cdiv(N, 128), T_t = p2w_cdiv(M, 128) * nNt1;
        gemm_hp_sk_kernel<PREC, 2, 2, 2, 2><<<8 * p2w_cdiv(T_t * sk_S, 8), 256, 0, stream>>>(Ah, ldh_a, Wp, M, Kpad, nNt1, T_t, sk_S, skws);
        gemm_hp_skfix_kernel<PREC, 2, 2, 2, 2><<<T_t * 4, 256, 0, stream>>>(skws, T_t, sk_S, nslab, nNt1, wscale, M, N, ep, o, ef);
    } else if (t64) {
        const int nMt = p2w_cdiv(M, 64), nNt1 = p2w_cdiv(N, 128);
        const int tm = pick_mode(nNt1, nMt, 3), nvb = tile_grid(nMt, nNt1, tm);
        gemm_hp64_kernel<PREC><<<pgrid(nvb, 3), 256, 0, stream>>>(Ah, ldh_a, Wp, wscale, M, N, Kpad, nMt, nNt1, nvb, ep, o, ef, tm);
    } else if (big) {
        const int nMt = p2w_cdiv(M, 256), nNt2 = Npad / 256;
        const int tm = pick_mode(nNt2, nMt, 1), nvb = tile_grid(nMt, nNt2, tm);
        if (dotw) gemm_hp_kernel<PREC, 2, 4, 4, 2, true><<<pgrid(nvb, 1), 512, 0, stream>>>(Ah, ldh_a, Wp, wscale, M, N, Kpad, nMt, nNt2, nvb, ep, o, ef, tm);
        else gemm_hp_kernel<PREC, 2, 4, 4, 2><<<pgrid(nvb, 1), 512, 0, stream>>>(Ah, ldh_a, Wp, wscale, M, N, Kpad, nMt, nNt2, nvb, ep, o, ef, tm);
    } else {
        const int nMt = p2w_cdiv(M, 128), nNt1 = p2w_cdiv(N, 128);
        const int tm = pick_mode(nNt1, nMt, 2), nvb = tile_grid(nMt, nNt1, tm);
        if (dotw) gemm_hp_kernel<PREC, 2, 2, 2, 2, true><<<pgrid(nvb, 2), 256, 0, stream>>>(Ah, ldh_a, Wp, wscale, M, N, Kpad, nMt, nNt1, nvb, ep, o, ef, tm);
        else gemm_hp_kernel<PREC, 2, 2, 2, 2><<<pgrid(nvb, 2), 256, 0, stream>>>(Ah, ldh_a, Wp, wscale, M, N, Kpad, nMt, nNt1, nvb, ep, o, ef, tm);
    }
    return P2W_LAUNCH_STATUS();
}

template <int RT, int GPT> struct SaEpiRegs { float bias[2], s[2], t[2]; int dsc[RT][GPT]; };
template <int PREC, int RT, int G>
__device__ __forceinline__ void sa_epilogue_regs(const f32x16 (&acc)[RT][2], float wscale, int n0, int wc, int lane,
                                                 const SaEpiRegs<RT, 32 / G>& e, int C2, float* __restrict__ out, int ldo,
                                                 _Float16* __restrict__ out_h2, int ldh, float& amax) {
    static_assert(G == 32 || G == 8, "one or four targets per 32-row tile");
    constexpr int GPT = 32 / G;
    const int h = lane >> 5;
#pragma unroll
    for (int i = 0; i < RT; ++i) {
#pragma unroll
        for (int q = 0; q < GPT; ++q) {
            const int dsc = __builtin_amdgcn_readfirstlane(e.dsc[i][q]);
            if (dsc < 0) continue;
            const int tgt = dsc >> 6, d = dsc & 63;
#pragma unroll
            for (int j = 0; j < 2; ++j) {
                const int col = n0 + wc * 64 + j * 32 + (lane & 31);
                const bool cv = col < C2;
                const float sgn = e.s[j] < 0.f ? -1.f : 1.f;
                const fpair sg2 = {sgn, sgn};
                float ext;
                if constexpr (G == 32) {
                    if (d >= 32) {
                        fpair p[8];
#pragma unroll
                        for (int u = 0; u < 8; ++u) p[u] = fpair{acc[i][j][2 * u], acc[i][j][2 * u + 1]} * sg2;
                        float m0 = fmaxf(fmaxf(p[0][0], p[0][1]), p[1][0]);
                        float m1 = fmaxf(fmaxf(p[1][1], p[2][0]), p[2][1]);
                        float m2 = fmaxf(fmaxf(p[3][0], p[3][1]), p[4][0]);
                        float m3 = fmaxf(fmaxf(p[4][1], p[5][0]), p[5][1]);
                        m0 = fmaxf(fmaxf(m0, p[6][0]), p[6][1]);
                        m1 = fmaxf(fmaxf(m1, p[7][0]), p[7][1]);
                        ext = fmaxf(fmaxf(m0, m1), fmaxf(m2, m3));
                    } else {
                        ext = -INFINITY;
#pragma unroll
                        for (int r = 0; r < 16; ++r) {
                            const int slot = (r & 3) + 8 * (r >> 2) + 4 * h;
                            if (slot < d) ext = fmaxf(ext, sgn * acc[i][j][r]);
                        }
                    }
                } else {
                    ext = -INFINITY;
#pragma unroll
                    for (int r = 0; r < 4; ++r) {
                        const int slot = r + 4 * h;
                        if (slot < d) ext = fmaxf(ext, sgn * acc[i][j][4 * q + r]);
                    }
                }
                {
                    const auto sw = __builtin_amdgcn_permlane32_swap(__float_as_uint(ext), __float_as_uint(ext), false, false);
                    ext = fmaxf(__uint_as_float(sw[0]), __uint_as_float(sw[1]));
                }
                float vmax = fmaf(fmaxf(fmaf(sgn * ext, wscale, e.bias[j]), 0.f), e.s[j], e.t[j]);
                if (d == 0 || !cv) vmax = 0.f;
                amax = nan_max(amax, fabsf(vmax));
                if (cv && h == 0 && out) out[(size_t)tgt * ldo + col] = vmax;
                if (out_h2) {
                    const float nb = __uint_as_float(__builtin_amdgcn_update_dpp(0, __float_as_uint(vmax), 0xB1, 0xf, 0xf, false));
                    if (h == 0 && (lane & 1) == 0 && col < ldh) h_store2<PREC>(out_h2, ldh, tgt, col, vmax, nb);
                }
            }
        }
    }
}

template <int PREC, int BN, int RT, int G>
__global__ __launch_bounds__(512, 2) void sa_conv16p_kernel(const float* __restrict__ P, int ldp, const int* __restrict__ meta_j,
                                                            const float4* __restrict__ meta_g, const int* __restrict__ desc,
                                                            const int* __restrict__ tiles_dev, int M, const float* __restrict__ w1r4, int C1, int C1pad,
                                                            const _Float16* __restrict__ W2h, size_t plane, float wscale, int C2,
                                                            int nMt_, int nNt, const float* __restrict__ b2,
                                                            const float* __restrict__ bn_s, const float* __restrict__ bn_t,
                                                            float* __restrict__ out, int ldo, _Float16* __restrict__ out_h2,
                                                            int ldh, unsigned* __restrict__ range) {
    constexpr int NP = HCfg<PREC>::planes;
    constexpr int WCn = BN / 64, BM = 32 * RT * (8 / WCn), NW = 8, NR = BM / 128;
    constexpr int GPT = 32 / G;
    if (tiles_dev) M = *tiles_dev;
    const int nMt = tiles_dev ? (M + BM / 32 - 1) / (BM / 32) : nMt_;
    if (M <= 0) return;
    constexpr int A_CH = 4 * NP * BM, STAGE_CH = A_CH + 4 * NP * BN;
    constexpr int NWI = 4;
    constexpr int NI = (4 * NP * BN) / 64 / NWI;
    static_assert(NI >= 1, "every issuing wave has at least one W2 DMA piece per slab");
    __shared__ __attribute__((aligned(16))) char S[2 * STAGE_CH * 16 + 4 * 512 * 4 + 3 * SA_EPI_COLS * 4];
    float* const Wr = reinterpret_cast<float*>(S + 2 * STAGE_CH * 16);
    float* const Ep = Wr + 4 * 512;
    const int tid = threadIdx.x, lane = tid & 63;
    for (int i = tid; i < 4 * C1pad; i += 512) Wr[i] = w1r4[i];
    for (int i = tid; i < C2; i += 512) { Ep[i] = b2[i]; Ep[SA_EPI_COLS + i] = bn_s[i]; Ep[2 * SA_EPI_COLS + i] = bn_t[i]; }
    const int wave = __builtin_amdgcn_readfirstlane(tid >> 6), wr = wave / WCn, wc = wave % WCn;
    const int nitems = nMt * nNt, nslab = C1pad / H_BK;
    int first, stride, limit;
    if ((gridDim.x & 7) == 0) {
        const int xcd = blockIdx.x & 7, slot = blockIdx.x >> 3, per = gridDim.x >> 3;
        const int chunk = (nitems + 7) >> 3;
        first = xcd * chunk + slot; stride = per; limit = min((xcd + 1) * chunk, nitems);
    } else {
        first = blockIdx.x; stride = gridDim.x; limit = nitems;
    }
    if (first >= limit) return;
    const int my_items = (limit - first + stride - 1) / stride;
    const int total = my_items * nslab;
// ... 176 lines not shown
                for (int t = 0; t < RT; ++t) afq[kk][p][t] = *reinterpret_cast<const h8*>(st + (offA[t] ^ (kk << 5) ^ (p << 6)));
#pragma unroll
                for (int t = 0; t < 2; ++t) bfq[kk][p][t] = *reinterpret_cast<const h8*>(st + (offB[t] ^ (kk << 5) ^ (p << 6)));
            }
#pragma unroll
        for (int kk = 0; kk < 2; ++kk) {
            auto& af = afq[kk];
            auto& bf = bfq[kk];
#pragma unroll
            for (int i = 0; i < RT; ++i)
#pragma unroll
                for (int j = 0; j < 2; ++j) {
                    if constexpr (PREC == 0) {
                        acc[i][j] = h_mfma<PREC>(af[1][i], bf[0][j], acc[i][j]);
                        acc[i][j] = h_mfma<PREC>(af[0][i], bf[1][j], acc[i][j]);
                    }
                    acc[i][j] = h_mfma<PREC>(af[0][i], bf[0][j], acc[i][j]);
                }
            if (kk == 0) {
                produce((g + 1) & 1, ma, k_of(c1), va, wk);
                constexpr int NM = 2 * RT * (PREC == 0 ? 3 : 1);
#pragma unroll
                for (int q = 0; q < NM; ++q) {
                    __builtin_amdgcn_sched_group_barrier(0x008, 1, 0);
                    __builtin_amdgcn_sched_group_barrier(0x002, (PREC == 0 ? 16 : 40) * NR / RT, 0);
                }
                __builtin_amdgcn_sched_barrier(0);
            }
        }
#pragma unroll
        for (int u = 0; u < NR; ++u) {
            asm volatile("" : "+v"(vb.v[u][0].x), "+v"(vb.v[u][0].y), "+v"(vb.v[u][0].z), "+v"(vb.v[u][0].w),
                              "+v"(vb.v[u][1].x), "+v"(vb.v[u][1].y), "+v"(vb.v[u][1].z), "+v"(vb.v[u][1].w));
            asm volatile("" : "+v"(mc.j[u]), "+v"(mc.g[u].x), "+v"(mc.g[u].y), "+v"(mc.g[u].z), "+v"(mc.g[u].w));
        }
#pragma unroll
        for (int i = 0; i < RT; ++i)
#pragma unroll
            for (int q = 0; q < GPT; ++q) asm volatile("" : "+v"(dg_n.d[i][q]));
        __builtin_amdgcn_s_waitcnt(p2w_vmcnt_imm(0));
        if (c0.s == nslab - 1) {
            SaEpiRegs<RT, GPT> e;
#pragma unroll
            for (int j = 0; j < 2; ++j) {
                const int col = min(c0.nt * BN + wc * 64 + j * 32 + (lane & 31), C2 - 1);
                e.bias[j] = Ep[col]; e.s[j] = Ep[SA_EPI_COLS + col]; e.t[j] = Ep[2 * SA_EPI_COLS + col];
            }
#pragma unroll
            for (int i = 0; i < RT; ++i)
#pragma unroll
                for (int q = 0; q < GPT; ++q) e.dsc[i][q] = (c0.mt * (BM / 32) + wr * RT + i >= M) ? -1 : dg_.d[i][q];
            sa_epilogue_regs<PREC, RT, G>(acc, wscale, c0.nt * BN, wc, lane, e, C2, out, ldo, out_h2, ldh, amax);
#pragma unroll
            for (int i = 0; i < RT; ++i)
#pragma unroll
                for (int j = 0; j < 2; ++j)
#pragma unroll
                    for (int e2 = 0; e2 < 16; ++e2) acc[i][j][e2] = 0.f;
        }
        __builtin_amdgcn_sched_barrier(0);
        va = vb; ma = mb; mb = mc; dg_ = dg_n;
        c0 = c1; c1 = c2; c2 = c3; c3 = nxt(c3);
    }
    if (range) range_commit_max(range, amax, lane);
}


__global__ __launch_bounds__(256) void sa_edge_meta_kernel(const float4* __restrict__ xyzr, const int* __restrict__ idx, const int* __restrict__ batch_dst,
                                    const float* __restrict__ sf, const int* __restrict__ nbr, const int* __restrict__ deg, int kw,
                                    int M, int n_src, int ldp4, int G, const int* __restrict__ list, const int* __restrict__ n_list_dev,
                                    const int* __restrict__ src_row, int* __restrict__ meta_j, float4* __restrict__ meta_g, int* __restrict__ desc,
                                    float4* __restrict__ zero_row);
constexpr int SA_PART_BLOCK = 1024;
__global__ __launch_bounds__(SA_PART_BLOCK) void sa_part_count_kernel(const int* __restrict__ deg, int kw, int M, int* __restrict__ blk_small);
__global__ __launch_bounds__(1024) void sa_part_scan_kernel(int* __restrict__ blk_small, int nblk, int M, int* __restrict__ counts);
__global__ __launch_bounds__(SA_PART_BLOCK) void sa_part_scatter_kernel(const int* __restrict__ deg, int kw, int M, const int* __restrict__ blk_small,
                                                                     int* __restrict__ list_small, int* __restrict__ list_large);

static inline size_t sa_conv_ws_bytes(long M, int flags) {
    const long tiles32 = M, tiles8 = (M + 3) / 4;
    if (!(flags & P2W_SA_PACK8)) return (size_t)(tiles32 * 32 * 20 + tiles32 * 4 + 256);
    const long nblk = (M + SA_PART_BLOCK - 1) / SA_PART_BLOCK;
    return (size_t)((tiles32 + tiles8) * 32 * 20 + (tiles32 + tiles8 * 4) * 4 + 2 * M * 4 + nblk * 4 + 64 + 1024);
}

template <int PREC>
static int32_t launch_sa_conv_h(const float* P, int32_t ldp, int32_t n_src, const float* xyzr_src, const int32_t* idx, const int32_t* batch_dst,
                                const float* sf, const int32_t* nbr, const int32_t* deg, int32_t kw, int32_t M,
                                const float* w1r4, const _Float16* W2h, float wscale, int32_t C1, int32_t C2, const float* b2,
                                const float* bn_s, const float* bn_t, float* out, int32_t ldo, _Float16* out_h2, int32_t ldh,
                                void* ws, size_t ws_bytes, int32_t flags, hipStream_t stream, const int32_t* src_row = nullptr,
                                unsigned* range = nullptr) {
    constexpr int KA = HCfg<PREC>::kalign;
    const int C2pad = (C2 + 255) / 256 * 256, C1pad = (C1 + KA - 1) / KA * KA;
    if (C1pad > 512 || C2 > SA_EPI_COLS || (long)M >= (1L << 25) || ((long)n_src + 1) * (ldp / 4) >= (1L << 31)) return P2W_EUNSUPPORTED;
    if (ldp < C1pad) return P2W_EINVAL;
    if (ws == nullptr || ws_bytes < sa_conv_ws_bytes(M, flags)) return P2W_EWORKSPACE;
    if (reinterpret_cast<uintptr_t>(ws) & 15u) return P2W_EALIGN;
    const int n_cu = p2w_cu_count();
    const bool wide = (flags & (P2W_SA_ITEM_256 | P2W_SA_ITEM_128)) ? (flags & P2W_SA_ITEM_256) != 0 : C2 > 128;
    const int tpi = wide ? 4 : 8, nNt3 = p2w_cdiv(C2, wide ? 256 : 128);
    const float4* x4 = reinterpret_cast<const float4*>(xyzr_src);
    auto run = [&](auto g_c, const int* list, const int* n_list_dev, const int* tiles_dev, long tiles_max, float4* meta_g, int* meta_j,
                   int* desc) {
        constexpr int G = decltype(g_c)::value;
        const long rows_max = tiles_max * 32;
        sa_edge_meta_kernel<<<p2w_cdiv(rows_max, 256), 256, 0, stream>>>(x4, idx, batch_dst, sf, nbr, deg, kw, M, n_src, ldp / 4, G,
                                                                       list, n_list_dev, src_row, meta_j, meta_g, desc,
                                                                       reinterpret_cast<float4*>(const_cast<float*>(P) + (size_t)n_src * ldp));
        const long items = p2w_cdiv(tiles_max, tpi) * nNt3;
        int grid = (int)(items < n_cu ? items : n_cu);
        if (grid >= 8) grid &= ~7;
        const int nMt3 = (int)p2w_cdiv(tiles_max, tpi);
        if (wide)
            sa_conv16p_kernel<PREC, 256, 2, G><<<grid, 512, 0, stream>>>(
                P, ldp, meta_j, meta_g, desc, tiles_dev, (int)tiles_max, w1r4, C1, C1pad, W2h, (size_t)C2pad * C1pad, wscale, C2, nMt3,
                nNt3, b2, bn_s, bn_t, out, ldo, out_h2, ldh, range);
        else
            sa_conv16p_kernel<PREC, 128, 2, G><<<grid, 512, 0, stream>>>(
                P, ldp, meta_j, meta_g, desc, tiles_dev, (int)tiles_max, w1r4, C1, C1pad, W2h, (size_t)C2pad * C1pad, wscale, C2, nMt3,
                nNt3, b2, bn_s, bn_t, out, ldo, out_h2, ldh, range);
    };
    char* w = static_cast<char*>(ws);
    if (!(flags & P2W_SA_PACK8)) {
        float4* meta_g = reinterpret_cast<float4*>(w);
        int* meta_j = reinterpret_cast<int*>(meta_g + (size_t)M * 32);
        int* desc = meta_j + (size_t)M * 32;
        run(std::integral_constant<int, 32>{}, nullptr, nullptr, nullptr, M, meta_g, meta_j, desc);
        return P2W_LAUNCH_STATUS();
    }
    const long t32 = M, t8 = (M + 3) / 4, nblk = p2w_cdiv(M, SA_PART_BLOCK);
    float4* mg_l = reinterpret_cast<float4*>(w);            w += t32 * 32 * 16;
    float4* mg_s = reinterpret_cast<float4*>(w);            w += t8 * 32 * 16;
    int* mj_l = reinterpret_cast<int*>(w);                  w += t32 * 32 * 4;
    int* mj_s = reinterpret_cast<int*>(w);                  w += t8 * 32 * 4;
    int* desc_l = reinterpret_cast<int*>(w);                w += t32 * 4;
    int* desc_s = reinterpret_cast<int*>(w);                w += t8 * 4 * 4;
    int* list_s = reinterpret_cast<int*>(w);                w += (size_t)M * 4;
    int* list_l = reinterpret_cast<int*>(w);                w += (size_t)M * 4;
    int* blk = reinterpret_cast<int*>(w);                   w += nblk * 4;
    int* counts = reinterpret_cast<int*>(w);
    sa_part_count_kernel<<<(int)nblk, SA_PART_BLOCK, 0, stream>>>(deg, kw, M, blk);
    sa_part_scan_kernel<<<1, 1024, 0, stream>>>(blk, (int)nblk, M, counts);
    sa_part_scatter_kernel<<<(int)nblk, SA_PART_BLOCK, 0, stream>>>(deg, kw, M, blk, list_s, list_l);
    run(std::integral_constant<int, 8>{}, list_s, counts + 0, counts + 2, t8, mg_s, mj_s, desc_s);
    run(std::integral_constant<int, 32>{}, list_l, counts + 1, counts + 3, t32, mg_l, mj_l, desc_l);
    return P2W_LAUNCH_STATUS();
}

int32_t p2w_gemm_h1_impl(int32_t prec, const _Float16* Ah, int32_t ldh_a, const _Float16* Wp, float wscale, int32_t M, int32_t N,
                         int32_t K, const EpiArgs& ep, float* out_f32, int32_t ldo, _Float16* out_h2, int32_t ldh_o,
                         int32_t flags, hipStream_t stream, const float* dotw = nullptr, float* part = nullptr, int32_t ldpart = 0,
                         float* skws = nullptr, size_t skws_bytes = 0);
int32_t p2w_sa_conv_h1_impl(int32_t prec, const float* P, int32_t ldp, int32_t n_src, const float* xyzr_src, const int32_t* idx,
                            const int32_t* batch_dst, const float* sf, const int32_t* nbr, const int32_t* deg, int32_t kw,
                            int32_t M, const float* w1r4, const _Float16* W2h, float wscale, int32_t C1, int32_t C2,
                            const float* b2, const float* bn_s, const float* bn_t, float* out, int32_t ldo, _Float16* out_h2,
                            int32_t ldh, void* ws, size_t ws_bytes, int32_t flags, hipStream_t stream, const int32_t* src_row = nullptr,
                            unsigned* range = nullptr);
```

### pointstowood_amd/engine.py

```python
from __future__ import annotations

import contextlib
import ctypes as C
import math
from dataclasses import dataclass, field, fields

import torch

from . import _lib
from ._lib import GEMM_RESIDUAL_H, PREC_F16X3, PREC_OF, SA_PACK8, SEARCH_BOX, SEARCH_Q_ROW_IN_W, SEARCH_X_INDEX_IN_W, Epilogue, check, lib, ptr

BN_EPS = 1e-5
SA_RES = (0.04, 0.08, 0.16)


@dataclass
class Linear:
    w: torch.Tensor
    N: int
    K: int
    bias: torch.Tensor | None = None
    sc0: torch.Tensor | None = None
    sh0: torch.Tensor | None = None
    sc1: torch.Tensor | None = None
# ... 119 lines not shown
class Level:
    xyzr: torch.Tensor
    ptr: torch.Tensor
    batch: torch.Tensor
    idx: torch.Tensor | None = None
    nbr: torch.Tensor | None = None
    deg: torch.Tensor | None = None
    n: int = -1


@dataclass
class Geometry:
    B: int
    N: int
    k: int
    sf: torch.Tensor
    levels: list = field(default_factory=list)
    fp_nbr: dict = field(default_factory=dict)
    counts_dev: torch.Tensor | None = None
    counts_host: torch.Tensor | None = None
    done: object = None
    args: tuple = ()
    stream: object = None
    search_stream: object = None
    table_levels: list = field(default_factory=list)
    table_probes: list = field(default_factory=list)
    order: torch.Tensor | None = None
    sorted0: torch.Tensor | None = None
    rows0_sorted: bool = False
    order64: torch.Tensor | None = None
    inv0: torch.Tensor | None = None
    pstride: int = 0
    sizes_ready: object = None
    ev_nbr: dict = field(default_factory=dict)
    ev_fp: dict = field(default_factory=dict)
    aux: list = field(default_factory=list)
    launch_searches: object = None
    early: dict | None = None
    watch: object = None
    lone: bool = False

    def tensors(self):
        out = [self.sf, self.counts_dev]
        for lv in self.levels:
            out += [t for t in (lv.xyzr, lv.ptr, lv.batch, lv.idx, lv.nbr, lv.deg) if t is not None]
        for nbr, deg in self.fp_nbr.values():
            out += [nbr, deg]
        out += self.aux + list(self.args)
        return [t for t in out if t is not None]


@dataclass(frozen=True)
class HLayout:
    slab: int
    planes: int
    dtype: torch.dtype

    def pitch(self, f):
        return (f + self.slab - 1) // self.slab * self.slab

    def new(self, rows, f, dev):
        return torch.empty((rows, self.planes * self.pitch(f)), dtype=self.dtype, device=dev)

    def col(self, t, c):
        return t[:, self.planes * c:]


class TableProvision:
    CELLS_MAX = 1 << 26
    SCALE_MAX = 64
    REST = 64

    def __init__(self, options):
        self.options = options
        self.scale = [1, 1, 1]
        self.rest = [0, 0, 0]
        self.probe_rest = [0, 0, 0]

    def cells(self, level, B, N):
        if self.options.sampler != "table":
            return 0, False
        if self.rest[level] > 0:
            self.rest[level] -= 1
            return 0, False
        per_voxel = (int(2.3 / SA_RES[level]) + 3) ** 3
        if B * per_voxel > self.options.table_cells_per_point * max(N, 1):
            return 0, False
        cells = B * per_voxel * self.scale[level]
        if cells <= self.CELLS_MAX:
            return cells, False
        if self.probe_rest[level] > 0:
            self.probe_rest[level] -= 1
            return 0, False
        s = self.scale[level]
        while s > 1 and B * per_voxel * s > self.CELLS_MAX:
            s //= 8
        cells = B * per_voxel * s
        return (cells, True) if cells <= self.CELLS_MAX else (0, False)

    def overflowed(self, level, was_probe):
        if was_probe:
            self.probe_rest[level] = self.REST
            return
        if self.scale[level] >= self.SCALE_MAX:
            self.rest[level] = self.REST
        self.scale[level] = min(self.scale[level] * 8, self.SCALE_MAX)


def pick_chunk(m: int, budget: int, col_tiles: int, n_cu: int = 256, full_rounds: bool = False) -> int:
    if m <= 0:
        return 256
    budget = max(256, budget // 256 * 256)
    if m <= budget * 5 // 4:
        per_round = max(256, 256 * n_cu // max(1, col_tiles) // 256 * 256)
        tiles = -(-m // 256) * col_tiles
        rounds_ = -(-tiles // n_cu)
        if full_rounds and m > per_round and tiles * 100 < rounds_ * n_cu * 78:
            return m // per_round * per_round
        return -(-m // 256) * 256
    best, best_cost = budget, None
    lo, hi = max(256, budget * 3 // 5 // 256 * 256), budget * 5 // 4 // 256 * 256
    for c in range(lo, hi + 1, 256):
        full, rem = divmod(m, c)
        rounds = lambda rows: -(-(-(-rows // 256) * col_tiles) // n_cu)
        cost = full * rounds(c) + (rounds(rem) if rem else 0)
        if best_cost is None or cost < best_cost or (cost == best_cost and c > best):
            best, best_cost = c, cost
    return best


@dataclass
class EngineOptions:
    sampler: str = "table"
    search: str = "grid"
    table_cells_per_point: float = 32.0
    search_index: bool = True
    search_box: int = 0
    fp1_cell_order: bool = False
    fp_hints: bool = True
    sa_pack: bool = True
    chunk_pick: bool = True
    chunk_full_rounds: bool = True
    res_chunk_rows: int = 131072
    res_streams: int = 1
    feature_streams: int = 2
    geo_priority: int = 0
    feat_priority: int = -1
    res_priority: int = -1
    gemm_flags: int = 0
    fp_hoist: bool = True
    fp_hoist_ratio: float = 0.5
    range_guard: bool = True
    gemm_stream_k: bool = True
    sa_flags: int = 0
    overlap: bool = True
    search_priority: int = 0
    search_stagger: bool = False
    early_first: bool = True
    table_prepared: bool = True
    single_res_streams: int = 2

    def __post_init__(self):
        if self.sampler not in ("table", "sort"):
            raise ValueError("sampler must be 'table' or 'sort'")
        if self.search not in ("grid", "brute"):
            raise ValueError("search must be 'grid' or 'brute'")

    @classmethod
    def names(cls):
        return tuple(f.name for f in fields(cls))


class Engine:
    def __init__(self, weights: PackedWeights, k: int = 32, precision: str = "f16x3", options: EngineOptions | None = None, **kw):
        self.w = weights
        self.k = int(k)
        if precision not in ("f16x3", "fp32", "fp16", "bf16"):
            raise ValueError("precision must be 'f16x3' (split-fp16 MFMA, fp32-class accuracy: the parity default), 'fp32' "
                             "(fp32 MFMA), or 'fp16' / 'bf16' (one MFMA per product: the reference's autocast arithmetic, "
                             "does not meet the 1e-4 probability bar)")
        if getattr(weights, "precision", precision) != precision:
            raise ValueError(f"weights were packed for precision {weights.precision!r}, not {precision!r}")
        self.precision = precision
        self.prec = PREC_OF.get(precision)
        if not 1 <= self.k <= 32:
            raise ValueError("k must be in 1..32: the fused PointNetConv maps a target's neighbour slots onto one 32-row MFMA "
                             "tile (P2W_MAX_K_CONV in include/p2w.h); the reference hard-codes k = 32 (model.py:210-212)")
        if options is not None and kw:
            raise TypeError("pass either options= or individual EngineOptions fields")
        self.options = options if options is not None else EngineOptions(**kw)
        for name in EngineOptions.names():
            setattr(self, name, getattr(self.options, name))
        self.h = {"f16x3": HLayout(32, 2, torch.float16), "fp16": HLayout(64, 1, torch.float16), "bf16": HLayout(64, 1, torch.bfloat16)}.get(precision)
        self._table = TableProvision(self)
        self._table_scale, self._table_rest, self._table_probe_rest = self._table.scale, self._table.rest, self._table.probe_rest
        self._side_streams = {}
        self._search_streams = {}
        self._sk_ws = {}
        self._zeros_c = {}
        self._s_geo = self._s_feat = None
        self._seen_warned = False
        self._ws_t = None
        self._range = None
        self.fallback = None
        self.range_fallbacks = 0
        self._static_range = [(f"sa{l}.layer1", f"geometry weights up to {weights.sa[l - 1]['w1r_bound']:.3g}") for l in (1, 2, 3)
                              if self.prec == PREC_F16X3 and self.options.range_guard and weights.sa[l - 1].get("w1r_bound", 0.0) > self.W1R_LIMIT]
        self.events = None
        self.events_grouped = False
        self._open = None
        self.stem_out = None
        self._ws = None

    def _chains(self, geo):
        return max(1, int(self.single_res_streams if geo.lone else self.res_streams))

    @staticmethod
    def _companion(pool, priority):
        key = _lib.stream()
        if key not in pool:
            pool[key] = torch.cuda.Stream(priority=int(priority))
        return pool[key]

    def _chunk_chains(self, geo, M, width, col_tiles, full_rounds, lane_bufs, body):
        chunk = (self.res_chunk_rows if self.res_chunk_rows > 0 else M) * 512 // width
        chunk = max(256, min(M, pick_chunk(M, chunk, col_tiles, full_rounds=full_rounds and self.chunk_full_rounds and not self.gemm_stream_k)
                             if self.chunk_pick else chunk // 256 * 256))
        cur = torch.cuda.current_stream()
        lanes = [cur]
        if min(self._chains(geo), -(-M // chunk)) > 1:
            lanes.append(self._companion(self._side_streams, self.res_priority))
        bufs = [lane_bufs(min(M, chunk)) for _ in lanes]
        if len(lanes) > 1:
            ready = torch.cuda.Event()
            ready.record(cur)
            lanes[1].wait_event(ready)
        for ci, r0 in enumerate(range(0, M, chunk)):
            with torch.cuda.stream(lanes[ci % len(lanes)]):
                body(r0, min(chunk, M - r0), bufs[ci % len(lanes)])
        if len(lanes) > 1:
            done = torch.cuda.Event()
            done.record(lanes[1])
            cur.wait_event(done)

    def _call(self, name, fn, *args):
        ev = self.events
        if ev is None:
            check(fn(*args, _lib.stream()), name)
            return
        if self.events_grouped:
            if self._open is not None and self._open[0] == name:
                check(fn(*args, _lib.stream()), name)
                self._open[3] += 1
                return
            self.flush_events()
            s = torch.cuda.Event(enable_timing=True)
            s.record()
            check(fn(*args, _lib.stream()), name)
            self._open = [name, s, None, 1]
            return
        s, e = torch.cuda.Event(enable_timing=True), torch.cuda.Event(enable_timing=True)
        s.record()
        check(fn(*args, _lib.stream()), name)
        e.record()
        ev.append((name, s, e))

    def flush_events(self):
        if self._open is not None:
            e = torch.cuda.Event(enable_timing=True)
            e.record()
            self._open[2] = e
            self.events.append(tuple(self._open))
            self._open = None

    @staticmethod
    def _epilogue(lin: Linear, residual=None, ldr=0, *watch_interp):
        return Epilogue(ptr(lin.bias), ptr(lin.sc0), ptr(lin.sh0), ptr(lin.sc1), ptr(lin.sh1), ptr(residual), ldr,
                        lin.relu0, lin.relu1, lin.relu2, lin.relu_final, *watch_interp)

    def _gemm(self, name, A, lda, M, lin: Linear, out, ldo, residual=None, ldr=0):
        ep = self._epilogue(lin, residual, ldr)
        self._call(name, lib().p2w_gemm, ptr(A), lda, ptr(lin.w), M, lin.N, lin.K, C.byref(ep), ptr(out), ldo)

    def _table_workspace(self, n, cells, device):
        need = int(lib().p2w_voxel_sample_table_ws_bytes(n, cells))
        if need == 0:
            raise RuntimeError("p2w_voxel_sample_table_ws_bytes failed")
        if self._ws_t is None or self._ws_t.numel() < need or self._ws_t.device != device:
            self._ws_t = torch.empty(need, dtype=torch.uint8, device=device)
            check(lib().p2w_voxel_sample_table_prepare(ptr(self._ws_t), self._ws_t.numel(), _lib.stream()), "voxel_sample_table_prepare")
        return self._ws_t

    def _workspace(self, n, device):
        need = int(lib().p2w_voxel_sample_ws_bytes(n))
        if need == 0:
            raise RuntimeError("p2w_voxel_sample_ws_bytes failed (no usable HIP device?)")
        if self._ws is None or self._ws.numel() < need or self._ws.device != device:
            self._ws = torch.empty(need, dtype=torch.uint8, device=device)
        return self._ws

    def _geometry_async(self, pos, reflectance, ptr0, sf, force_sort: bool = False, search_stream=None, defer_searches: bool = False) -> Geometry:
        L = lib()
        dev = pos.device
        N, B, k = pos.shape[0], sf.numel(), self.k
        i32 = dict(dtype=torch.int32, device=dev)
        f32 = dict(dtype=torch.float32, device=dev)
# ... 91 lines not shown
                           ptr(lv.idx), ptr(lv.ptr), B, N, k, ptr(lv.nbr), ptr(lv.deg), None,
                           (SEARCH_BOX if self.search_box & 2 else 0))
            else:
                self._call("knn", L.p2w_knn, ptr(src.xyzr), ptr(src.ptr), ptr(src.xyzr), ptr(lv.idx), ptr(lv.ptr), B, N,
                           k, ptr(lv.nbr), ptr(lv.deg), ptr(boxes(l)), 0)
            mark(geo.ev_nbr, l + 1)

        def fp_search(f):
            fine, coarse = geo.levels[f], geo.levels[f + 1]
            nbr, deg = geo.fp_nbr[f]
            q, fl = (sorted0, 0 if geo.rows0_sorted else SEARCH_Q_ROW_IN_W) if f == 0 else (fine.xyzr, 0)
            if grid_search:
                hint = hints.get(f)
                if hint is not None:
                    self._call("knn_hint", L.p2w_knn_hint2, ptr(q), ptr(ranks[f]), ptr(fine.ptr), B, N, ptr(coarse.xyzr),
                               ptr(hint))
                self._call("knn2", L.p2w_knn_grid_indexed, ptr(coarse.xyzr), ptr(ckeys[f + 1]), ptr(coarse.ptr), ptr(grids[f + 1]),
                           ptr(cstart.get(f + 1)), ptr(q), None, ptr(fine.ptr), B, N, 2, ptr(nbr), ptr(deg), ptr(hint),
                           fl | (SEARCH_BOX if self.search_box & 4 else 0))
            else:
                self._call("knn2", L.p2w_knn, ptr(coarse.xyzr), ptr(coarse.ptr), ptr(q), None, ptr(fine.ptr), B, N, 2,
                           ptr(nbr), ptr(deg), ptr(boxes(f + 1)), fl)
            mark(geo.ev_fp, f)
        jobs = [lambda l=l: sa_search(l) for l in range(3)] + [lambda f=f: fp_search(f) for f in (2, 1, 0)]

        def launch_searches(count=None, after=None):
            first = len(jobs) == 6
            todo = jobs[: (len(jobs) if count is None else count)]
            del jobs[: len(todo)]
            if first and search_stream is not None:
                search_stream.wait_event(geo.sizes_ready)
            if after is not None and search_stream is not None:
                search_stream.wait_event(after)
            with torch.cuda.stream(search_stream) if search_stream is not None else contextlib.nullcontext():
                for job in todo:
                    job()
                if not jobs:
                    geo.launch_searches, geo.done = None, torch.cuda.Event()
                    geo.done.record()
        aux0 += [box0, cstart0, geo.inv0, geo.order64]
        for d in (bbox, hints, ckeys, grids, ranks, cstart):
            aux0 += d.values()
        geo.aux = [t for t in aux0 if t is not None]
        geo.launch_searches = launch_searches
        if not defer_searches:
            launch_searches()
        return geo

    def _geometry_finish(self, geo):
        geo.sizes_ready.synchronize()
        ps = geo.pstride
        overflow = [l for l in geo.table_levels if int(geo.counts_host[3 * ps + l])]
        if overflow:
            for l in overflow:
                self._table.overflowed(l, l in geo.table_probes)
            with torch.cuda.stream(geo.stream):
                if geo.search_stream is not None:
                    if geo.launch_searches is not None:
                        geo.launch_searches()
                    geo.stream.wait_event(geo.done)
                geo = self._geometry_async(*geo.args, force_sort=True, search_stream=geo.search_stream)
            geo.sizes_ready.synchronize()
        for l in (1, 2, 3):
            geo.levels[l].n = int(geo.counts_host[(l - 1) * geo.pstride + geo.B])
        return geo

    def geometry(self, pos, reflectance, ptr0, sf) -> Geometry:
        return self._geometry_finish(self._geometry_async(pos, reflectance, ptr0, sf))

    def features(self, geo: Geometry, keep: dict | None = None):
        if self.prec is not None:
            if geo.early is None:
                self._range_begin(geo.sf.device)
            logits = self._features_h2(geo, keep)
            geo.watch = self._range_end()
            return logits
        geo.watch = None
        if geo.search_stream is not None:
            if geo.launch_searches is not None:
                geo.launch_searches()
            torch.cuda.current_stream().wait_event(geo.done)
        return self._features_fp32(geo, keep)

    def checked(self, geo: Geometry, logits, keep: dict | None = None):
        bad = self.range_violations(geo.watch)
        if not bad:
            return logits
        what = "; ".join(f"{n}: {v}" for n, v in bad[:4])
        sampled_only = all(v.startswith("no value above") for _, v in bad)
        if sampled_only and (self.fallback is None or geo.rows0_sorted):
            if not self._seen_warned:
                import warnings
                self._seen_warned = True
                warnings.warn(f"pointstowood_amd: precision {self.precision!r}: the range watch saw no value above {self.RANGE_LO:g} in its "
                              f"sample of {what} and no fp32 recomputation is available in this configuration: logits returned as computed")
            return logits
        if self.fallback is None:
            raise RuntimeError(f"precision {self.precision!r}: activations outside the range of the 16-bit planes ({what}); "
                               "use precision='fp32'")
        if self.range_fallbacks == 0:
            import warnings
            warnings.warn(f"pointstowood_amd: precision {self.precision!r} cannot carry this checkpoint's activations ({what}): such "
                          "batches are recomputed on the fp32 MFMA path (about 4x slower)")
        self.range_fallbacks += 1
        return self.fallback(geo, keep)

    RANGE_SLOTS = 64
    RANGE_WORDS = 1024
    RANGE_HI, RANGE_LO = 6.0e4, 2.0 ** -5
    W1R_LIMIT = 65504.0 - 6.0e4

    def _watch(self, layer, rows=1):
        w = self._range
        if w is None or layer is None or rows <= 0:
            return None
        names, buf = w
        if layer not in names:
            if len(names) >= self.RANGE_SLOTS:
                return None
            names.append(layer)
        return buf.data_ptr() + 4 * self.RANGE_WORDS * names.index(layer)

    def _range_begin(self, dev):
        self._range = ([], torch.zeros(self.RANGE_SLOTS * self.RANGE_WORDS, dtype=torch.int32, device=dev)) if (self.range_guard and self.prec == PREC_F16X3) else None

    def _range_end(self):
        w, self._range = self._range, None
        if w is None:
            return None
        host = torch.empty(2 * self.RANGE_SLOTS, dtype=torch.int32, pin_memory=True)
        host.copy_(w[1].view(self.RANGE_SLOTS, self.RANGE_WORDS // 64, 64)[:, :, :2].amax(dim=1).reshape(-1), non_blocking=True)
        return w[0], w[1], host

    def range_violations(self, watch):
        if watch is None:
            return []
        names, _, host = watch
        bad = list(self._static_range)
        flags = host[: 2 * len(names)].tolist()
        for i, n in enumerate(names):
            if flags[2 * i]:
                bad.append((n, f"values beyond +-{self.RANGE_HI:g} (or NaN)"))
            elif not flags[2 * i + 1]:
                bad.append((n, f"no value above {self.RANGE_LO:g}"))
        return bad

    def _gemm_h2(self, name, A, ldh_a, M, lin: Linear, out_f32=None, ldo=0, out_h2=None, ldh_o=0, residual=None, ldr=0,
                 residual_h=False, watch=None, interp=None):
        ep = self._epilogue(lin, residual, ldr, self._watch(watch, M), ptr(interp), 0 if interp is None else residual.shape[0])
        flags = self.gemm_flags | (GEMM_RESIDUAL_H if residual_h else 0)
        if self.gemm_stream_k:
            ws = self._sk_workspace(A.device)
            self._call(name, lib().p2w_gemm_h2_sk, self.prec, ptr(A), ldh_a, ptr(lin.w16), lin.wscale, M, lin.N, lin.K, C.byref(ep),
                       ptr(out_f32), ldo, ptr(out_h2), ldh_o, ptr(ws), ws.numel(), flags)
            return
        self._call(name, lib().p2w_gemm_h2, self.prec, ptr(A), ldh_a, ptr(lin.w16), lin.wscale, M, lin.N, lin.K, C.byref(ep),
                   ptr(out_f32), ldo, ptr(out_h2), ldh_o, flags)

    def _sk_workspace(self, dev):
        key = _lib.stream()
        ws = self._sk_ws.get(key)
        if ws is None:
            ws = self._sk_ws[key] = torch.empty(int(lib().p2w_gemm_h2_sk_ws_bytes()), dtype=torch.uint8, device=dev)
        return ws

    def _hoist(self, xh_src, pitch_src, n_src, p, l):
        C1, C1p = p["C1"], self.h.pitch(p["C1"])
        P = torch.empty((n_src + 1, C1p), dtype=torch.float32, device=xh_src.device)
        if C1p != C1:
            P[:, C1:].zero_()
        self._gemm_h2("gemm_hoist", xh_src, pitch_src, n_src, p["hoist"], out_f32=P, ldo=C1p, watch=f"hoist{l}")
        return P

    def _features_early(self, geo: Geometry):
        L, w = lib(), self.w
        dev = geo.sf.device
        Cw, N, prec = w.C, geo.N, self.prec
        F3 = 16 * Cw
        pitch0 = self.h.pitch(F3 + Cw)
        cat0 = self.h.new(N, F3 + Cw, dev)
        xh0 = self.h.col(cat0, F3)
        x0 = torch.empty((N, Cw), dtype=torch.float32, device=dev)
        stem, rec0 = (L.p2w_stem_h2_indexed, geo.sorted0) if geo.rows0_sorted else (L.p2w_stem_h2, geo.levels[0].xyzr)
        self._call("stem", stem, prec, ptr(rec0), N, ptr(w.stem_w), ptr(w.stem_b), Cw, ptr(x0), ptr(xh0), pitch0, self._watch("stem", N))
        self.stem_out = x0
        P1 = self._hoist(xh0, pitch0, N, w.sa[0], 1)
        return dict(lv0=geo.levels[0], cat0=cat0, x0=x0, P1=P1)

    def _features_h2(self, geo: Geometry, keep: dict | None = None):
        L, w = lib(), self.w
        dev = geo.sf.device
        Cw = w.C
        new = lambda r, c: torch.empty((r, c), dtype=torch.float32, device=dev)
        prec = self.prec
        pad8, hcol = self.h.pitch, self.h.col
        newh = lambda r, f: self.h.new(r, f, dev)
        lv, N, B = geo.levels, geo.N, geo.B
        F3 = 16 * Cw
        res_h = prec == PREC_F16X3
        Fs = [Cw, 4 * Cw, 8 * Cw, 16 * Cw]
        rows = [N, lv[1].n, lv[2].n, lv[3].n]
        pitch = [pad8(F3 + Fs[f]) for f in range(4)]
        early = geo.early or self._features_early(geo)
        cat = [early["cat0"]] + [newh(rows[f], F3 + Fs[f]) for f in range(1, 4)]
        xh = [hcol(cat[f], F3) for f in range(4)]
        x0 = early["x0"]
        sorted0 = geo.rows0_sorted
        wait = lambda ev: torch.cuda.current_stream().wait_event(ev) if ev is not None else None

        def need(table, key):
            while table.get(key) is None and geo.launch_searches is not None:
                geo.launch_searches(1)
            wait(table.get(key))

        def stage(count):
            if geo.launch_searches is not None and geo.search_stream is not None:
                ev = torch.cuda.Event()
                ev.record()
                geo.launch_searches(count, after=ev)
        if keep is not None:
            keep["stem"] = x0
        x3 = None
        for l in (1, 2, 3):
            p, src, dst = w.sa[l - 1], lv[l - 1], lv[l]
            M, C1, C2, E = dst.n, p["C1"], p["C2"], 4 * p["C2"]
            C1p = pad8(C1)
            P = early["P1"] if l == 1 else self._hoist(xh[l - 1], pitch[l - 1], src.n, p, l)
            need(geo.ev_nbr, l)
            conv = new(M, C2) if (keep is not None or not res_h) else None
            convh = newh(M, C2)
            sa_flags = self.sa_flags | (SA_PACK8 if (l == 1 and self.sa_pack) else 0)
            meta = torch.empty(int(L.p2w_sa_conv_h_ws_bytes(M, sa_flags)) + 65536, dtype=torch.uint8, device=dev)
            if keep is not None:
                keep[f"sa{l}_module.ws"] = meta
            self._call("sa_conv", L.p2w_sa_conv_h_rows, prec, ptr(P), C1p, src.n, ptr(src.xyzr), ptr(dst.idx), ptr(dst.batch),
                       ptr(geo.sf), ptr(dst.nbr), ptr(dst.deg), geo.k, M, ptr(p["w1r4"]), ptr(p["W2"].w16),
                       p["W2"].wscale, C1, C2, ptr(p["b2"]), ptr(p["bn_s"]), ptr(p["bn_t"]), ptr(conv), C2, ptr(convh),
                       pad8(C2), ptr(meta), meta.numel(), sa_flags, ptr(geo.inv0) if (l == 1 and sorted0) else None, self._watch(f"sa{l}", M))
            stage(1 if l < 3 else 2)
            out = new(M, C2) if (keep is not None or l == 3) else None
            def res_chunk(r0, m, bufs):
                e1, e2 = bufs
                self._gemm_h2("gemm_res", convh[r0:], pad8(C2), m, p["g1"], out_h2=e1, ldh_o=pad8(E), watch=f"res{l}.1")
                self._gemm_h2("gemm_res", e1, pad8(E), m, p["g2"], out_h2=e2, ldh_o=pad8(E), watch=f"res{l}.2")
                self._gemm_h2("gemm_res", e2, pad8(E), m, p["g3"], out_h2=e1, ldh_o=pad8(E), watch=f"res{l}.3")
                self._gemm_h2("gemm_res", e1, pad8(E), m, p["g4"], out_f32=None if out is None else out[r0:], ldo=C2,
                              out_h2=xh[l][r0:], ldh_o=pitch[l],
                              residual=convh[r0:] if res_h else conv[r0:], ldr=pad8(C2) if res_h else C2, residual_h=res_h,
                              watch=f"res{l}.4")
            self._chunk_chains(geo, M, E, E // 256, True, lambda rows: (newh(rows, E), newh(rows, E)), res_chunk)
            if l == 3:
                x3 = out
            if keep is not None:
                keep[f"sa{l}_module.conv"], keep[f"sa{l}_module.out"] = conv, out
        M3 = lv[3].n
        cat_g = newh(M3, F3 + 4)
        self._call("concat_xyz", L.p2w_concat_xyz_h2, prec, ptr(x3), F3, ptr(lv[3].xyzr), M3, ptr(cat_g), pad8(F3 + 4))
        h1, h2 = newh(M3, F3), new(M3, F3)
        self._gemm_h2("gemm_mlp", cat_g, pad8(F3 + 4), M3, w.sa4[0], out_h2=h1, ldh_o=pad8(F3), watch="sa4.0")
        self._gemm_h2("gemm_mlp", h1, pad8(F3), M3, w.sa4[1], out_f32=h2, ldo=F3, watch="sa4.1")
        g = new(B, F3)
        self._call("segment_max", L.p2w_segment_max, ptr(h2), F3, F3, ptr(lv[3].ptr), B, ptr(g))
        if keep is not None:
            keep["sa4_module.out"] = g
        nbr4 = torch.empty(M3, dtype=torch.int32, device=dev)
        deg4 = torch.empty(M3, dtype=torch.int32, device=dev)
        self._call("fill_batch_nbr", L.p2w_fill_batch_nbr, ptr(lv[3].batch), M3, ptr(nbr4), ptr(deg4))
        zc = self._zeros_c
        if (B, dev) not in zc:
            zc[(B, dev)] = torch.zeros((B, 4), dtype=torch.float32, device=dev)
            torch.cuda.current_stream().synchronize()
        zeros_c = zc[(B, dev)]
        y, y_xyzr, y_h = g, zeros_c, None
        y_rows, y_cols = g.shape
        logits = torch.empty(N, dtype=torch.float32, device=dev) if w.num_classes == 1 else None
        o_multi = new(N, w.num_classes) if w.num_classes != 1 else None
        logits_out = logits
        for fl in (4, 3, 2, 1):
            fine = lv[fl - 1]
            m, Fc, cf, ld = fine.n, y_cols, cat[fl - 1], pitch[fl - 1]
            nbr, deg, kw = (nbr4, deg4, 1) if fl == 4 else (*geo.fp_nbr[fl - 1], 2)
            if fl < 4:
                need(geo.ev_fp, fl - 1)
            fine_xyzr = geo.sorted0 if (fl == 1 and sorted0) else fine.xyzr
            l0, l1 = w.fp[fl]
            hoists = lambda rows_c, rows_f: bool(self.fp_hoist and 0 < rows_c <= self.fp_hoist_ratio * rows_f)
            Mx = y_rows
            hoist = hoists(Mx, m)
            next_hoist = fl >= 2 and hoists(m, lv[fl - 2].n)
            if hoist:
                li, ls = w.fp_split[fl]
                if y_h is None:
                    y_h = newh(Mx, Fc + 4)
                    self._call("concat_xyz", L.p2w_concat_xyz_h2, prec, ptr(y), Fc, ptr(y_xyzr), Mx, ptr(y_h), pad8(Fc + 4))
                    y_ld = pad8(Fc + 4)
                else:
                    y_ld = pad8(Fc)
                Z = new(Mx, l0.N)
                self._gemm_h2("gemm_mlp", y_h, y_ld, Mx, li, out_f32=Z, ldo=l0.N)
                rec = torch.empty((m, 4), dtype=torch.int32, device=dev)
                self._call("interp_concat", L.p2w_interp_weights, ptr(y_xyzr), ptr(fine_xyzr), ptr(nbr), ptr(deg), kw, m, ptr(rec))
            yh_full = newh(m, l1.N) if next_hoist else None
            need_f32 = (fl > 1 and not next_hoist) or keep is not None
            b = new(m, l1.N) if need_f32 else None
            one = fl == 1 and w.num_classes == 1

            def fp_bufs(mc):
                return dict(a=newh(mc, l0.N), yh=newh(mc, l1.N) if fl == 1 else None,
                            hws=torch.empty(int(L.p2w_gemm_h2_rowdot_ws_bytes(mc, w.head1.N)), dtype=torch.uint8, device=dev) if one else None,
                            hdh=newh(mc, F3) if (fl == 1 and not one) else None)

            def fp_chunk(r0, mm, bf):
                a, yh, hws, hdh = bf["a"], bf["yh"], bf["hws"], bf["hdh"]
                if hoist:
                    self._gemm_h2("gemm_mlp", xh[fl - 1][r0:], ld, mm, ls, out_h2=a, ldh_o=pad8(l0.N), residual=Z, ldr=l0.N,
                                  interp=rec[r0:], watch=f"fp{fl}.0")
                else:
                    self._call("interp_concat", L.p2w_interp_concat_h2, prec, ptr(y), Fc, ptr(y_xyzr), ptr(fine_xyzr[r0:]),
                               ptr(nbr[r0:]), ptr(deg[r0:]), kw, None, 0, mm, ptr(cf[r0:]), ld)
                    self._gemm_h2("gemm_mlp", cf[r0:], ld, mm, l0, out_h2=a, ldh_o=pad8(l0.N), watch=f"fp{fl}.0")
                if yh_full is not None:
                    yh = yh_full[r0:]
                self._gemm_h2("gemm_mlp", a, pad8(l0.N), mm, l1, out_f32=None if b is None else b[r0:], ldo=l1.N,
                              out_h2=yh, ldh_o=pad8(l1.N), watch=f"fp{fl}.1")
                if one:
                    lin, ep = w.head1, self._epilogue(w.head1)
                    self._call("gemm_mlp", L.p2w_gemm_h2_rowdot, prec, ptr(yh), pad8(F3), ptr(lin.w16), lin.wscale, mm, lin.N,
                               lin.K, C.byref(ep), ptr(w.head2_w), float(w.head2_b[0]), ptr(logits[r0:]), ptr(hws),
                               hws.numel(), self.gemm_flags)
                elif fl == 1:
                    self._gemm_h2("gemm_mlp", yh, pad8(F3), mm, w.head1, out_h2=hdh, ldh_o=pad8(F3), watch="head1")
                    self._gemm_h2("gemm_mlp", hdh, pad8(F3), mm, w.head2, out_f32=o_multi[r0:], ldo=w.num_classes)
            self._chunk_chains(geo, m, Fc + Fs[fl - 1], max(1, l0.N // 256), False, fp_bufs, fp_chunk)
            y, y_xyzr, y_h = b, fine.xyzr, yh_full
            y_rows, y_cols = m, l1.N
            if keep is not None:
                if fl == 1 and sorted0 and b is not None:
                    bo = torch.empty_like(b)
                    bo[geo.order64] = b
                    b = bo
                keep[f"fp{fl}_module.out"] = b
        if sorted0:
            if w.num_classes == 1:
                logits_out = torch.empty_like(logits)
                logits_out[geo.order64] = logits
                logits = logits_out
            else:
                om = torch.empty_like(o_multi)
                om[geo.order64] = o_multi
                o_multi = om
        if w.num_classes != 1:
            logits = o_multi.t()
        return torch.squeeze(logits)

    def _features_fp32(self, geo: Geometry, keep: dict | None = None):
        L, w = lib(), self.w
        dev = geo.sf.device
        Cw = w.C
        new = lambda r, c: torch.empty((r, c), dtype=torch.float32, device=dev)
        lv = geo.levels
        N = geo.N
        x = [new(N, Cw)]
        self._call("stem", L.p2w_stem, ptr(lv[0].xyzr), N, ptr(w.stem_w), ptr(w.stem_b), Cw, ptr(x[0]))
        self.stem_out = x[0]
        if keep is not None:
            keep["stem"] = x[0]
        for l in (1, 2, 3):
            p, src, dst = w.sa[l - 1], lv[l - 1], lv[l]
            M, C1, C2, E = dst.n, p["C1"], p["C2"], 4 * p["C2"]
            P = new(src.n, C1)
            self._gemm("gemm_hoist", x[l - 1], p["F_in"], src.n, p["hoist"], P, C1)
            conv = new(M, C2)
            self._call("sa_conv", L.p2w_sa_conv, ptr(P), C1, ptr(src.xyzr), ptr(dst.idx), ptr(dst.batch), ptr(geo.sf),
                       ptr(dst.nbr), ptr(dst.deg), geo.k, M, ptr(p["w1r4"]), ptr(p["W2"].w), C1, C2, ptr(p["b2"]),
                       ptr(p["bn_s"]), ptr(p["bn_t"]), ptr(conv), C2)
            e1, e2 = new(M, E), new(M, E)
            self._gemm("gemm_res", conv, C2, M, p["g1"], e1, E)
            self._gemm("gemm_res", e1, E, M, p["g2"], e2, E)
            self._gemm("gemm_res", e2, E, M, p["g3"], e1, E)
            out = new(M, C2)
            self._gemm("gemm_res", e1, E, M, p["g4"], out, C2, residual=conv, ldr=C2)
            x.append(out)
            if keep is not None:
                keep[f"sa{l}_module.conv"], keep[f"sa{l}_module.out"] = conv, out
        F3, M3, B = 16 * Cw, lv[3].n, geo.B
        cat = new(M3, F3 + 4)
        self._call("concat_xyz", L.p2w_concat_xyz, ptr(x[3]), F3, ptr(lv[3].xyzr), M3, ptr(cat), F3 + 4)
        h1, h2 = new(M3, F3), new(M3, F3)
        self._gemm("gemm_mlp", cat, F3 + 4, M3, w.sa4[0], h1, F3)
        self._gemm("gemm_mlp", h1, F3, M3, w.sa4[1], h2, F3)
        g = new(B, F3)
        self._call("segment_max", L.p2w_segment_max, ptr(h2), F3, F3, ptr(lv[3].ptr), B, ptr(g))
        if keep is not None:
            keep["sa4_module.out"] = g
        nbr4 = torch.empty(M3, dtype=torch.int32, device=dev)
        deg4 = torch.empty(M3, dtype=torch.int32, device=dev)
        self._call("fill_batch_nbr", L.p2w_fill_batch_nbr, ptr(lv[3].batch), M3, ptr(nbr4), ptr(deg4))
        zeros_c = torch.zeros((B, 4), dtype=torch.float32, device=dev)
        y, y_xyzr = g, zeros_c
        for fl in (4, 3, 2, 1):
            fine = lv[fl - 1]
            m, Fc, Fs = fine.n, y.shape[1], x[fl - 1].shape[1]
# ... 118 lines not shown
```

Before: 20.51 million.

## Chain consecutive residual GEMMs in one persistent kernel with row-tile dependency counters

Adds a chained GEMM kernel that runs the third and fourth residual-block GEMMs in a single persistent launch. Each row tile of the second GEMM starts once all column tiles of that row from the first GEMM have finished, tracked by atomic counters in a control workspace. The aim is to remove a kernel boundary and the tail idle time between the two dependent GEMMs, and to let the second GEMM read the intermediate while it is still cache-resident. The cost is added synchronisation complexity: atomics, L2 writeback fences, and a control area that must be zeroed. Rows beyond the chained portion fall back to the two separate GEMMs.

```diff
diff --git a/include/p2w.h b/include/p2w.h
--- a/include/p2w.h
+++ b/include/p2w.h
@@ -212,6 +212,7 @@
 #define P2W_GEMM_NO_STREAMK 128
 #define P2W_GEMM_TILE_64 (1 << 24)
 #define P2W_GEMM_NO_TILE_64 (1 << 25)
+#define P2W_GEMM_CHAIN (1 << 26)
 #define P2W_SA_ITEM_256 1
 #define P2W_SA_ITEM_128 2
 #define P2W_SA_PACK8 4
@@ -223,6 +224,12 @@
 int32_t p2w_gemm_h2_sk(int32_t prec, const void* A_h, int32_t ldh_a, const void* Wh, float wscale, int32_t M, int32_t N,
                        int32_t K, const p2w_epilogue* epi, float* out_f32, int32_t ldo, void* out_h, int32_t ldh_o,
                        void* ws, size_t ws_bytes, int32_t flags, p2w_stream_t stream);
+size_t p2w_gemm_h2_chain_ws_bytes(void);
+int32_t p2w_gemm_h2_chain_rows(int32_t prec, int32_t M, int32_t N0, int32_t K0, int32_t N1, int32_t flags);
+int32_t p2w_gemm_h2_chain(int32_t prec, const void* A_h, int32_t ldh_a, const void* W0, float wscale0, int32_t M, int32_t N0,
+                          int32_t K0, const p2w_epilogue* epi0, void* e_h, int32_t ldh_e, int32_t flags0, const void* W1,
+                          float wscale1, int32_t N1, const p2w_epilogue* epi1, float* out_f32, int32_t ldo, void* out_h,
+                          int32_t ldh_o, int32_t flags1, void* ws, size_t ws_bytes, p2w_stream_t stream);
 size_t p2w_gemm_h2_rowdot_ws_bytes(int32_t M, int32_t N);
 int32_t p2w_gemm_h2_rowdot(int32_t prec, const void* A_h, int32_t ldh_a, const void* Wh, float wscale, int32_t M, int32_t N,
                            int32_t K, const p2w_epilogue* epi, const float* dot_w, float dot_b, float* out, void* ws,
diff --git a/pointstowood_amd/_lib.py b/pointstowood_amd/_lib.py
--- a/pointstowood_amd/_lib.py
+++ b/pointstowood_amd/_lib.py
@@ -22,6 +22,7 @@
 PREC_OF = {"f16x3": PREC_F16X3, "fp16": PREC_F16, "bf16": PREC_BF16}
 GEMM_TILE_128, GEMM_TILE_256, GEMM_GENERIC_EPI, GEMM_ORDER_ROWS, GEMM_ORDER_COLS, GEMM_RESIDUAL_H = 1, 2, 4, 8, 16, 32
 GEMM_STREAMK, GEMM_NO_STREAMK = 64, 128
+GEMM_CHAIN = 1 << 26
 SA_ITEM_256, SA_ITEM_128, SA_PACK8 = 1, 2, 4
 CLUSTER_LINK, CLUSTER_COMPRESS, CLUSTER_NUMBER, CLUSTER_ALL = 1, 2, 4, 7
 MAX_K_WIDE = 100
@@ -89,6 +90,10 @@
     "p2w_gemm_h2": (_i32, [_i32, _vp, _i32, _vp, _f32, _i32, _i32, _i32, C.POINTER(Epilogue), _vp, _i32, _vp, _i32, _i32, _vp]),
     "p2w_gemm_h2_sk_ws_bytes": (_sz, []),
     "p2w_gemm_h2_sk": (_i32, [_i32, _vp, _i32, _vp, _f32, _i32, _i32, _i32, C.POINTER(Epilogue), _vp, _i32, _vp, _i32, _vp, _sz, _i32, _vp]),
+    "p2w_gemm_h2_chain_ws_bytes": (_sz, []),
+    "p2w_gemm_h2_chain_rows": (_i32, [_i32, _i32, _i32, _i32, _i32, _i32]),
+    "p2w_gemm_h2_chain": (_i32, [_i32, _vp, _i32, _vp, _f32, _i32, _i32, _i32, C.POINTER(Epilogue), _vp, _i32, _i32, _vp, _f32, _i32,
+                                 C.POINTER(Epilogue), _vp, _i32, _vp, _i32, _i32, _vp, _sz, _vp]),
     "p2w_gemm_h2_rowdot_ws_bytes": (_sz, [_i32, _i32]),
     "p2w_gemm_h2_rowdot": (_i32, [_i32, _vp, _i32, _vp, _f32, _i32, _i32, _i32, C.POINTER(Epilogue), _vp, _f32, _vp, _vp, _sz, _i32, _vp]),
     "p2w_sa_conv_h_ws_bytes": (_sz, [_i32, _i32]),
diff --git a/pointstowood_amd/csrc/p2w_feat.hip b/pointstowood_amd/csrc/p2w_feat.hip
--- a/pointstowood_amd/csrc/p2w_feat.hip
+++ b/pointstowood_amd/csrc/p2w_feat.hip
@@ -305,9 +305,10 @@
     return P2W_LAUNCH_STATUS();
 }
 
-static int32_t gemm_h2_checked(int32_t prec, const void* A_h, int32_t ldh_a, const void* Wh, float wscale, int32_t M, int32_t N,
-                               int32_t K, const p2w_epilogue* epi, float* out_f32, int32_t ldo, void* out_h, int32_t ldh_o,
-                               void* ws, size_t ws_bytes, int32_t flags, p2w_stream_t stream) {
+static int32_t gemm_h2_args(int32_t prec, const void* A_h, int32_t ldh_a, const void* Wh, float wscale, int32_t M, int32_t N,
+                            int32_t K, const p2w_epilogue* epi, float* out_f32, int32_t ldo, void* out_h, int32_t ldh_o,
+                            void* ws, int32_t flags, EpiArgs* ep_out, bool* launch) {
+    *launch = false;
     if (prec < P2W_PREC_F16X3 || prec > P2W_PREC_BF16) return P2W_EINVAL;
     if (ws) P2W_CHECK_ALIGN16(ws);
     if ((flags & P2W_GEMM_STREAMK) && (flags & P2W_GEMM_NO_STREAMK)) return P2W_EINVAL;
@@ -339,6 +340,13 @@
             ep.residual = nullptr;
         }
     }
+    *ep_out = ep;
+    *launch = true;
+    return P2W_OK;
+}
+static int32_t gemm_h2_run(int32_t prec, const void* A_h, int32_t ldh_a, const void* Wh, float wscale, int32_t M, int32_t N, int32_t K,
+                           const EpiArgs& ep, float* out_f32, int32_t ldo, void* out_h, int32_t ldh_o, void* ws, size_t ws_bytes,
+                           int32_t flags, p2w_stream_t stream) {
     const _Float16* Ah = static_cast<const _Float16*>(A_h);
     const _Float16* Wp = static_cast<const _Float16*>(Wh);
     if (prec == P2W_PREC_F16X3)
@@ -347,6 +355,15 @@
     return p2w_gemm_h1_impl(prec, Ah, ldh_a, Wp, wscale, M, N, K, ep, out_f32, ldo, static_cast<_Float16*>(out_h), ldh_o, flags,
                             p2w_s(stream), nullptr, nullptr, 0, static_cast<float*>(ws), ws_bytes);
 }
+static int32_t gemm_h2_checked(int32_t prec, const void* A_h, int32_t ldh_a, const void* Wh, float wscale, int32_t M, int32_t N,
+                               int32_t K, const p2w_epilogue* epi, float* out_f32, int32_t ldo, void* out_h, int32_t ldh_o,
+                               void* ws, size_t ws_bytes, int32_t flags, p2w_stream_t stream) {
+    EpiArgs ep;
+    bool launch;
+    const int32_t rc = gemm_h2_args(prec, A_h, ldh_a, Wh, wscale, M, N, K, epi, out_f32, ldo, out_h, ldh_o, ws, flags, &ep, &launch);
+    if (rc != P2W_OK || !launch) return rc;
+    return gemm_h2_run(prec, A_h, ldh_a, Wh, wscale, M, N, K, ep, out_f32, ldo, out_h, ldh_o, ws, ws_bytes, flags, stream);
+}
 extern "C" int32_t p2w_gemm_h2(int32_t prec, const void* A_h, int32_t ldh_a, const void* Wh, float wscale, int32_t M, int32_t N,
                                int32_t K, const p2w_epilogue* epi, float* out_f32, int32_t ldo, void* out_h, int32_t ldh_o,
                                int32_t flags, p2w_stream_t stream) {
@@ -358,6 +375,57 @@
                                   void* ws, size_t ws_bytes, int32_t flags, p2w_stream_t stream) {
     if (!ws && ws_bytes) return P2W_ENULL;
     return gemm_h2_checked(prec, A_h, ldh_a, Wh, wscale, M, N, K, epi, out_f32, ldo, out_h, ldh_o, ws, ws_bytes, flags, stream);
+}
+
+extern "C" size_t p2w_gemm_h2_chain_ws_bytes(void) { return p2w_gemm_h2_sk_ws_bytes() + P2W_CHAIN_CTL_BYTES; }
+static int32_t chain_rows_of(int32_t prec, int32_t M, int32_t N0, int32_t K0, int32_t N1, int32_t flags) {
+    if (prec == P2W_PREC_F16X3) return gemm_chain_rows<0>(M, N0, K0, N1, flags);
+    return prec == P2W_PREC_F16 || prec == P2W_PREC_BF16 ? gemm_chain_rows<1>(M, N0, K0, N1, flags) : 0;
+}
+extern "C" int32_t p2w_gemm_h2_chain_rows(int32_t prec, int32_t M, int32_t N0, int32_t K0, int32_t N1, int32_t flags) {
+    return M > 0 && N0 > 0 && K0 > 0 && N1 > 0 ? chain_rows_of(prec, M, N0, K0, N1, flags) : 0;
+}
+extern "C" int32_t p2w_gemm_h2_chain(int32_t prec, const void* A_h, int32_t ldh_a, const void* W0, float wscale0, int32_t M, int32_t N0,
+                                     int32_t K0, const p2w_epilogue* epi0, void* e_h, int32_t ldh_e, int32_t flags0, const void* W1,
+                                     float wscale1, int32_t N1, const p2w_epilogue* epi1, float* out_f32, int32_t ldo, void* out_h,
+                                     int32_t ldh_o, int32_t flags1, void* ws, size_t ws_bytes, p2w_stream_t stream) {
+    if (!ws && ws_bytes) return P2W_ENULL;
+    EpiArgs ep0, ep1;
+    bool l0, l1;
+    int32_t rc = gemm_h2_args(prec, A_h, ldh_a, W0, wscale0, M, N0, K0, epi0, nullptr, 0, e_h, ldh_e, ws, flags0, &ep0, &l0);
+    if (rc != P2W_OK) return rc;
+    if (l0 && !e_h) return P2W_ENULL;
+    rc = gemm_h2_args(prec, e_h, ldh_e, W1, wscale1, M, N1, N0, epi1, out_f32, ldo, out_h, ldh_o, ws, flags1, &ep1, &l1);
+    if (rc != P2W_OK || !l0 || !l1) return rc;
+    const int PL = prec == P2W_PREC_F16X3 ? 2 : 1;
+    const size_t sk_bytes = p2w_gemm_h2_sk_ws_bytes();
+    int32_t rows = 0;
+    if (ws && ws_bytes >= sk_bytes + P2W_CHAIN_CTL_BYTES && !ep0.imeta && !ep1.imeta) rows = chain_rows_of(prec, M, N0, K0, N1, flags0);
+    const _Float16* Ah = static_cast<const _Float16*>(A_h);
+    _Float16* eh = static_cast<_Float16*>(e_h);
+    _Float16* oh = static_cast<_Float16*>(out_h);
+    if (rows > 0) {
+        int* ctl = reinterpret_cast<int*>(static_cast<char*>(ws) + sk_bytes);
+        if (prec == P2W_PREC_F16X3)
+            rc = launch_gemm_chain_h<0>(Ah, ldh_a, static_cast<const _Float16*>(W0), wscale0, rows, N0, K0, ep0, eh, ldh_e, flags0,
+                                        static_cast<const _Float16*>(W1), wscale1, N1, ep1, out_f32, ldo, oh, ldh_o, flags1, ctl, p2w_s(stream));
+        else
+            rc = p2w_gemm_chain_h1_impl(prec, Ah, ldh_a, static_cast<const _Float16*>(W0), wscale0, rows, N0, K0, ep0, eh, ldh_e, flags0,
+                                        static_cast<const _Float16*>(W1), wscale1, N1, ep1, out_f32, ldo, oh, ldh_o, flags1, ctl, p2w_s(stream));
+        if (rc != P2W_OK || rows == M) return rc;
+    }
+    const size_t r0 = (size_t)rows;
+    auto behind = [&](EpiArgs ep) {
+        if (ep.residual) ep.residual += r0 * ep.ldr;
+        if (ep.res_h) ep.res_h += r0 * PL * ep.ldr;
+        return ep;
+    };
+    const size_t skb = ws_bytes < sk_bytes ? ws_bytes : sk_bytes;
+    rc = gemm_h2_run(prec, Ah + r0 * PL * ldh_a, ldh_a, W0, wscale0, M - rows, N0, K0, behind(ep0), nullptr, 0, eh + r0 * PL * ldh_e, ldh_e,
+                     ws, skb, flags0, stream);
+    if (rc != P2W_OK) return rc;
+    return gemm_h2_run(prec, eh + r0 * PL * ldh_e, ldh_e, W1, wscale1, M - rows, N1, N0, behind(ep1), out_f32 ? out_f32 + r0 * ldo : nullptr, ldo,
+                       oh ? oh + r0 * PL * ldh_o : nullptr, ldh_o, ws, skb, flags1, stream);
 }
 
 __global__ __launch_bounds__(256) void rowdot_finish_kernel(const float* __restrict__ part, int ldpart, int nslots, float b, int M,
diff --git a/pointstowood_amd/csrc/p2w_feat_h1.hip b/pointstowood_amd/csrc/p2w_feat_h1.hip
--- a/pointstowood_amd/csrc/p2w_feat_h1.hip
+++ b/pointstowood_amd/csrc/p2w_feat_h1.hip
@@ -7,6 +7,17 @@
     if (prec == P2W_PREC_F16)
         return launch_gemm_h<1>(Ah, ldh_a, Wp, wscale, M, N, K, ep, out_f32, ldo, out_h2, ldh_o, flags, stream, dotw, part, ldpart, skws, skws_bytes);
     return launch_gemm_h<2>(Ah, ldh_a, Wp, wscale, M, N, K, ep, out_f32, ldo, out_h2, ldh_o, flags, stream, dotw, part, ldpart, skws, skws_bytes);
+}
+
+int32_t p2w_gemm_chain_h1_impl(int32_t prec, const _Float16* Ah, int32_t ldh_a, const _Float16* W0, float wscale0, int32_t rows, int32_t N0,
+                               int32_t K0, const EpiArgs& ep0, _Float16* e_h, int32_t ldh_e, int32_t flags0, const _Float16* W1, float wscale1,
+                               int32_t N1, const EpiArgs& ep1, float* out_f32, int32_t ldo, _Float16* out_h2, int32_t ldh_o, int32_t flags1,
+                               int* ctl, hipStream_t stream) {
+    if (prec == P2W_PREC_F16)
+        return launch_gemm_chain_h<1>(Ah, ldh_a, W0, wscale0, rows, N0, K0, ep0, e_h, ldh_e, flags0, W1, wscale1, N1, ep1, out_f32, ldo, out_h2,
+                                      ldh_o, flags1, ctl, stream);
+    return launch_gemm_chain_h<2>(Ah, ldh_a, W0, wscale0, rows, N0, K0, ep0, e_h, ldh_e, flags0, W1, wscale1, N1, ep1, out_f32, ldo, out_h2,
+                                  ldh_o, flags1, ctl, stream);
 }
 
 int32_t p2w_sa_conv_h1_impl(int32_t prec, const float* P, int32_t ldp, int32_t n_src, const float* xyzr_src, const int32_t* idx,
diff --git a/pointstowood_amd/csrc/p2w_hgemm.h b/pointstowood_amd/csrc/p2w_hgemm.h
--- a/pointstowood_amd/csrc/p2w_hgemm.h
+++ b/pointstowood_amd/csrc/p2w_hgemm.h
@@ -400,10 +400,11 @@
     if constexpr (WAIT_OLDER) __builtin_amdgcn_s_waitcnt(p2w_vmcnt_imm(0));
 }
 
-template <int PREC, int WR, int WC, int RT, int CT, bool DOTK, bool SK>
+struct ChainArgs { const _Float16* W; float wscale; int N, nNt, ef; EpiArgs ep; OutArgs o; int* ctl; };
+template <int PREC, int WR, int WC, int RT, int CT, bool DOTK, bool SK, bool CHAIN = false>
 __device__ __forceinline__ void gemm_hp_body(const _Float16* __restrict__ A, int ldh_a, const _Float16* __restrict__ Wh, float wscale,
                                              int M, int N, int Kpad, int nMt, int nNt, int nvb, const EpiArgs& ep, const OutArgs& o,
-                                             int ef, int tmode, int sk_S, float* __restrict__ skws) {
+                                             int ef, int tmode, int sk_S, float* __restrict__ skws, const ChainArgs* ch = nullptr) {
     constexpr int KS = HCfg<PREC>::kslab;
     constexpr int BM = 32 * RT * WR, BN = 32 * CT * WC, NW = WR * WC;
     constexpr int A_CH = 8 * BM, STAGE_CH = A_CH + 8 * BN;
@@ -411,7 +412,7 @@
     constexpr int NWI = HALF ? NW / 2 : NW;
     constexpr int NI = STAGE_CH / 64 / NWI;
     static_assert(STAGE_CH % (64 * NWI) == 0, "stage must split evenly over the issuing waves");
-    __shared__ __attribute__((aligned(16))) char S[2 * STAGE_CH * 16];
+    __shared__ __attribute__((aligned(16))) char S[2 * STAGE_CH * 16 + (CHAIN ? 16 : 0)];
     const int tid = threadIdx.x, lane = tid & 63;
     const int wave = __builtin_amdgcn_readfirstlane(tid >> 6), wr = wave / WC, wc = wave % WC;
     const size_t a_pitch = (size_t)HCfg<PREC>::planes * ldh_a, w_pitch = (size_t)HCfg<PREC>::planes * Kpad;
@@ -425,6 +426,31 @@
     const int nslab = Kpad / KS;
     int L = blockIdx.x, mt, nt;
     int sk_s0 = 0, sk_s1 = 0, sk_piece = 0;
+    int* const c_lds = reinterpret_cast<int*>(S + 2 * STAGE_CH * 16);
+    const int c_grp = blockIdx.x & 7;
+    int c_kind = 0;
+    int c_sig = -1;
+    int c_held = -1;
+    bool c_want = CHAIN, c_first = true;
+    bool c_done = false;
+    int c_pa = -1, c_pb = -1, c_pnt = 0;
+    int n_kind = 0, n_mt = 0, n_nt = 0;
+    bool n_more = false;
+    auto chain_leave = [&]() {
+        if (tid == 0) {
+            const int gone = __hip_atomic_fetch_add(ch->ctl + 8 + c_grp, 1, __ATOMIC_RELAXED, __HIP_MEMORY_SCOPE_AGENT);
+            if (gone == (int)(gridDim.x >> 3) - 1) {
+                __hip_atomic_store(ch->ctl + c_grp, 0, __ATOMIC_RELAXED, __HIP_MEMORY_SCOPE_AGENT);
+                __hip_atomic_store(ch->ctl + 8 + c_grp, 0, __ATOMIC_RELAXED, __HIP_MEMORY_SCOPE_AGENT);
+            }
+        }
+    };
+    auto chain_arrive = [&](int row) {
+        int* cnt = ch->ctl + 16 + row;
+        if (__hip_atomic_fetch_add(cnt, 1, __ATOMIC_RELAXED, __HIP_MEMORY_SCOPE_AGENT) != nNt - 1) return -1;
+        __hip_atomic_store(cnt, 0, __ATOMIC_RELAXED, __HIP_MEMORY_SCOPE_AGENT);
+        return row;
+    };
     if constexpr (SK) {
         const int P = nvb * sk_S, per_xcd = (P + 7) >> 3;
         const int w = blockIdx.x >> 3;
@@ -435,19 +461,30 @@
         sk_s1 = (int)((long long)(j + 1) * nslab / sk_S);
         if (sk_s0 >= sk_s1) return;
         mt = r / nNt; nt = r - mt * nNt;
+    } else if constexpr (CHAIN) {
+        if (tid == 0) *c_lds = __hip_atomic_fetch_add(ch->ctl + c_grp, 1, __ATOMIC_RELAXED, __HIP_MEMORY_SCOPE_AGENT);
+        __syncthreads();
+        const int t0 = __builtin_amdgcn_readfirstlane(*c_lds);
+        mt = c_grp + 8 * (t0 / nNt); nt = t0 % nNt;
+        if (mt >= nMt) { chain_leave(); return; }
     } else if (!next_tile(L, mt, nt)) {
         return;
     }
 
     const _Float16* src[NI];
-    auto setup_src = [&](int mt_, int nt_) {
+    auto setup_src = [&](int mt_, int nt_, int kind_ = 0) {
+        const _Float16 *Ab = A, *Wb = Wh;
+        size_t ap = a_pitch, wp = w_pitch;
+        if constexpr (CHAIN) {
+            if (kind_) { Ab = o.h2; ap = (size_t)HCfg<PREC>::planes * o.ldh; Wb = ch->W; wp = (size_t)HCfg<PREC>::planes * N; }
+        }
 #pragma unroll
         for (int i = 0; i < NI; ++i) {
             const int g = (wave % NWI) + NWI * i;
             const int row = 8 * g + (lane >> 3);
             const int c = (lane & 7) ^ ((row >> 1) & 7);
-            if (g < BM / 8) src[i] = A + (size_t)min(mt_ * BM + row, M - 1) * a_pitch + 8 * c;
-            else src[i] = Wh + (size_t)(nt_ * BN + w_stage_row16(row - BM)) * w_pitch + 8 * c;
+            if (g < BM / 8) src[i] = Ab + (size_t)min(mt_ * BM + row, M - 1) * ap + 8 * c;
+            else src[i] = Wb + (size_t)(nt_ * BN + w_stage_row16(row - BM)) * wp + 8 * c;
         }
     };
     const unsigned lds_base = (unsigned)(uintptr_t)(lds_vp)S;
@@ -488,7 +525,38 @@
         landed = false;
         __builtin_amdgcn_s_barrier();
         asm volatile("" ::: "memory");
-        if constexpr (LAST) setup_src(mtn, ntn);
+        if constexpr (CHAIN) {
+            if (s == 1 && c_sig >= 0 && wave == NW - 1) asm volatile("buffer_wbl2 sc1" ::: "memory");
+            if (s == 2 && (c_sig >= 0 || c_want) && wave == NW - 1) {
+                asm volatile("s_waitcnt vmcnt(0)" ::: "memory");
+                if (lane == 0) {
+                    const int tk = c_want ? __hip_atomic_fetch_add(ch->ctl + c_grp, 1, __ATOMIC_RELAXED, __HIP_MEMORY_SCOPE_AGENT) : -1;
+                    const int own = c_sig >= 0 ? chain_arrive(c_sig) : -1;
+                    c_lds[0] = tk; c_lds[1] = own;
+                }
+            }
+            if constexpr (LAST) {
+                if (c_want) {
+                    c_held = __builtin_amdgcn_readfirstlane(c_lds[0]);
+                    if (c_grp + 8 * (c_held / nNt) >= nMt) { c_held = -1; c_done = true; }
+                }
+                if (c_sig >= 0) {
+                    const int own = __builtin_amdgcn_readfirstlane(c_lds[1]);
+                    if (own >= 0) { if (c_pa < 0) { c_pa = own; c_pnt = 0; } else c_pb = own; }
+                }
+                if (c_pa >= 0 && c_pnt >= ch->nNt) { c_pa = c_pb; c_pb = -1; c_pnt = 0; }
+                n_more = true;
+                if (c_pa >= 0) {
+                    if (c_pnt == 0 && issuer) __builtin_amdgcn_fence(__ATOMIC_ACQUIRE, "agent");
+                    n_kind = 1; n_mt = c_pa; n_nt = c_pnt++;
+                } else if (c_held >= 0) {
+                    n_kind = 0; n_mt = c_grp + 8 * (c_held / nNt); n_nt = c_held % nNt; c_held = -1;
+                } else {
+                    n_more = false; n_kind = c_kind; n_mt = mt; n_nt = nt;
+                }
+                setup_src(n_mt, n_nt, n_kind);
+            }
+        } else if constexpr (LAST) setup_src(mtn, ntn);
         constexpr int HR = RT16 / 2;
         constexpr int NG = 2 * HR * CT16;
         constexpr int GAP = (NG / (2 * NI)) > 0 ? NG / (2 * NI) : 1;
@@ -548,6 +616,47 @@
         for (int i = 0; i < RT16; ++i)
 #pragma unroll
             for (int j = 0; j < CT16; ++j) dst[(i * CT16 + j) * (64 * NW)] = acc[i][j];
+    } else if constexpr (CHAIN) {
+        const int nslab1 = N / KS;
+        while (true) {
+#pragma unroll
+            for (int i = 0; i < RT16; ++i)
+#pragma unroll
+                for (int j = 0; j < CT16; ++j) acc[i][j] = f32x4{0.f, 0.f, 0.f, 0.f};
+            const int ns = c_kind ? nslab1 : nslab;
+            for (int s = 0; s + 1 < ns; ++s) slab(s, std::false_type{}, 0, 0);
+            slab(ns - 1, std::true_type{}, 0, 0);
+            const int row0 = mt * BM + wr * 32 * RT, col0 = nt * BN + wc * 32 * CT;
+            if (c_kind) gemm_epilogue_dispatch16<PREC, RT16, CT16, true, false>(acc, ch->ep, ch->wscale, row0, col0, lane, M, ch->N, ch->o, ch->ef, wave == 0);
+            else gemm_epilogue_dispatch16<PREC, RT16, CT16, true, false>(acc, ep, wscale, row0, col0, lane, M, N, o, ef, c_first && wave == 0);
+            landed = true;
+            c_first = false;
+            c_sig = c_kind == 0 ? mt : -1;
+            if (!n_more) {
+                if (c_sig < 0) break;
+                asm volatile("s_waitcnt vmcnt(0)" ::: "memory");
+                __syncthreads();
+                if (wave == NW - 1) {
+                    __builtin_amdgcn_fence(__ATOMIC_RELEASE, "agent");
+                    asm volatile("s_waitcnt vmcnt(0)" ::: "memory");
+                    if (lane == 0) c_lds[1] = chain_arrive(c_sig);
+                }
+                __syncthreads();
+                const int own = __builtin_amdgcn_readfirstlane(c_lds[1]);
+                if (own < 0) break;
+                if (issuer) __builtin_amdgcn_fence(__ATOMIC_ACQUIRE, "agent");
+                c_pa = own; c_pnt = 1; c_sig = -1;
+                n_kind = 1; n_mt = own; n_nt = 0;
+                setup_src(n_mt, n_nt, n_kind);
+                if (issuer) {
+#pragma unroll
+                    for (int i = 0; i < NI; ++i) issue_piece(i, gs & 1, 0);
+                }
+                landed = false;
+            }
+            c_kind = n_kind; mt = n_mt; nt = n_nt;
+            c_want = c_kind == 0 && !c_done;
+        }
     } else {
     while (true) {
         int Ln = L + gridDim.x, mtn = mt, ntn = nt;
@@ -567,6 +676,7 @@
     }
     }
     asm volatile("s_waitcnt vmcnt(0)" ::: "memory");
+    if constexpr (CHAIN) chain_leave();
 }
 
 template <int PREC, int WR, int WC, int RT, int CT, bool DOTK = false>
@@ -575,6 +685,13 @@
                                                                int Kpad, int nMt, int nNt, int nvb, EpiArgs ep, OutArgs o, int ef,
                                                                int tmode) {
     gemm_hp_body<PREC, WR, WC, RT, CT, DOTK, false>(A, ldh_a, Wh, wscale, M, N, Kpad, nMt, nNt, nvb, ep, o, ef, tmode, 0, nullptr);
+}
+
+template <int PREC>
+__global__ __launch_bounds__(512, 2) void gemm_hp_chain_kernel(const _Float16* __restrict__ A, int ldh_a, const _Float16* __restrict__ Wh,
+                                                            float wscale, int M, int N, int Kpad, int nMt, int nNt, EpiArgs ep, OutArgs o,
+                                                            int ef, ChainArgs ch) {
+    gemm_hp_body<PREC, 2, 4, 4, 2, false, false, true>(A, ldh_a, Wh, wscale, M, N, Kpad, nMt, nNt, 0, ep, o, ef, 0, 0, nullptr, &ch);
 }
 
 template <int PREC>
@@ -611,6 +728,66 @@
     }
     const int mt = r / nNt, nt = r - mt * nNt;
     gemm_epilogue_dispatch16<PREC, 1, CT16, false, false>(acc, ep, wscale, mt * BM + wr * 32 * RT + 16 * i, nt * BN + wc * 32 * CT, lane, M, N, o, ef);
+}
+
+static inline int gemm_epi_class(const EpiArgs& ep, int32_t M, int32_t N, const float* out_f32, int32_t ldo, const _Float16* out_h2,
+                                 int32_t ldh_o, int32_t flags, const float* dotw = nullptr, const float* part = nullptr, int32_t ldpart = 0) {
+    int ef = (ep.relu0 ? 1 : 0) | (ep.sc0 ? 2 : 0) | (ep.relu1 ? 4 : 0) | (ep.sc1 ? 8 : 0) | (ep.relu2 ? 16 : 0) |
+             ((ep.residual || ep.res_h) ? 32 : 0) | (ep.relu_final ? 64 : 0) | (out_f32 ? 128 : 0) | (out_h2 ? 256 : 0) | (dotw ? 512 : 0) |
+             (ep.res_h ? 1024 : 0) | (ep.imeta ? 2048 : 0);
+    const size_t lim = (size_t)1 << 31;
+    if ((size_t)M * (size_t)(ldo > 2 * ldh_o ? ldo : 2 * ldh_o) >= lim || ((ep.residual || ep.res_h) && !ep.imeta && (size_t)M * (size_t)ep.ldr * (ep.res_h ? 2 : 1) >= lim) ||
+        (N & 1) || (flags & P2W_GEMM_GENERIC_EPI))
+        ef = 0;
+    auto odd8 = [](const void* q) { return (reinterpret_cast<uintptr_t>(q) & 7) != 0; };
+    if ((out_f32 && ((ldo & 1) || odd8(out_f32))) || (ep.residual && ((ep.ldr & 1) || odd8(ep.residual))) || odd8(ep.bias) ||
+        (ep.res_h && ((ep.ldr & 7) || (reinterpret_cast<uintptr_t>(ep.res_h) & 15))) ||
+        odd8(ep.sc0) || odd8(ep.sh0) || odd8(ep.sc1) || odd8(ep.sh1) || odd8(dotw) || (part && ((ldpart & 3) || (reinterpret_cast<uintptr_t>(part) & 15))))
+        ef = 0;
+    return ef;
+}
+
+constexpr int P2W_CHAIN_CTL_BYTES = 65536;
+template <int PREC>
+static inline int32_t gemm_chain_rows(int32_t M, int32_t N0, int32_t K0, int32_t N1, int32_t flags) {
+    constexpr int KA = HCfg<PREC>::kalign, KS = HCfg<PREC>::kslab;
+    if (!(flags & P2W_GEMM_CHAIN)) return 0;
+    if (M < 256 || N0 < 256 || (N0 % 256) || N0 > 2048 || N1 < 256 || (N1 % 256) || K0 <= 0) return 0;
+    const int Kpad0 = (K0 + KA - 1) / KA * KA;
+    if (Kpad0 / KS < 4 || N0 / KS < 4) return 0;
+    const int n_cu = p2w_cu_count(), nNt0 = N0 / 256;
+    if (n_cu < 8) return 0;
+    const long q = (long)(M / 256) * nNt0 / n_cu;
+    if (q < 1) return 0;
+    long mt_full = q * n_cu / nNt0;
+    const long cap = (P2W_CHAIN_CTL_BYTES / 4 - 16);
+    if (mt_full > cap) mt_full = cap;
+    return (int32_t)(mt_full * 256);
+}
+template <int PREC>
+static int32_t launch_gemm_chain_h(const _Float16* Ah, int32_t ldh_a, const _Float16* W0, float wscale0, int32_t rows, int32_t N0, int32_t K0,
+                                   const EpiArgs& ep0, _Float16* e_h, int32_t ldh_e, int32_t flags0, const _Float16* W1, float wscale1,
+                                   int32_t N1, const EpiArgs& ep1, float* out_f32, int32_t ldo, _Float16* out_h2, int32_t ldh_o,
+                                   int32_t flags1, int* ctl, hipStream_t stream) {
+    constexpr int KA = HCfg<PREC>::kalign;
+    const int Kpad0 = (K0 + KA - 1) / KA * KA;
+    if ((ldh_a % KA) != 0 || ldh_a < Kpad0 || (ldh_e % KA) != 0 || ldh_e < N0 || (ldh_e & 7) || (out_h2 && (ldh_o & 7))) return P2W_EINVAL;
+    const int hcols1 = ldh_o < (N1 + KA - 1) / KA * KA ? ldh_o : (N1 + KA - 1) / KA * KA;
+    const OutArgs o0 = {nullptr, 0, e_h, ldh_e, N0, nullptr, nullptr, 0};
+    ChainArgs ch;
+    ch.W = W1; ch.wscale = wscale1; ch.N = N1; ch.nNt = N1 / 256; ch.ep = ep1;
+    ch.o = OutArgs{out_f32, ldo, out_h2, ldh_o, hcols1, nullptr, nullptr, 0};
+    ch.ef = gemm_epi_class(ep1, rows, N1, out_f32, ldo, out_h2, ldh_o, flags1);
+    ch.ctl = ctl;
+    const int ef0 = gemm_epi_class(ep0, rows, N0, nullptr, 0, e_h, ldh_e, flags0);
+    const int nMt = rows / 256, nNt0 = N0 / 256;
+    const long tiles = (long)nMt * nNt0;
+    int grid = p2w_cu_count();
+    if (tiles < grid) grid = (int)tiles;
+    grid &= ~7;
+    if (grid < 8) return P2W_EINVAL;
+    gemm_hp_chain_kernel<PREC><<<grid, 512, 0, stream>>>(Ah, ldh_a, W0, wscale0, rows, N0, Kpad0, nMt, nNt0, ep0, o0, ef0, ch);
+    return P2W_LAUNCH_STATUS();
 }
 
 template <int PREC>
@@ -715,18 +892,7 @@
                                        best_mode == 2 ? skws : nullptr, skws_bytes, best_mode == 2 ? best_S : 0);
         }
     }
-    int ef = (ep.relu0 ? 1 : 0) | (ep.sc0 ? 2 : 0) | (ep.relu1 ? 4 : 0) | (ep.sc1 ? 8 : 0) | (ep.relu2 ? 16 : 0) |
-             ((ep.residual || ep.res_h) ? 32 : 0) | (ep.relu_final ? 64 : 0) | (out_f32 ? 128 : 0) | (out_h2 ? 256 : 0) | (dotw ? 512 : 0) |
-             (ep.res_h ? 1024 : 0) | (ep.imeta ? 2048 : 0);
-    const size_t lim = (size_t)1 << 31;
-    if ((size_t)M * (size_t)(ldo > 2 * ldh_o ? ldo : 2 * ldh_o) >= lim || ((ep.residual || ep.res_h) && !ep.imeta && (size_t)M * (size_t)ep.ldr * (ep.res_h ? 2 : 1) >= lim) ||
-        (N & 1) || (flags & P2W_GEMM_GENERIC_EPI))
-        ef = 0;
-    auto odd8 = [](const void* q) { return (reinterpret_cast<uintptr_t>(q) & 7) != 0; };
-    if ((out_f32 && ((ldo & 1) || odd8(out_f32))) || (ep.residual && ((ep.ldr & 1) || odd8(ep.residual))) || odd8(ep.bias) ||
-        (ep.res_h && ((ep.ldr & 7) || (reinterpret_cast<uintptr_t>(ep.res_h) & 15))) ||
-        odd8(ep.sc0) || odd8(ep.sh0) || odd8(ep.sc1) || odd8(ep.sh1) || odd8(dotw) || (part && ((ldpart & 3) || (reinterpret_cast<uintptr_t>(part) & 15))))
-        ef = 0;
+    const int ef = gemm_epi_class(ep, M, N, out_f32, ldo, out_h2, ldh_o, flags, dotw, part, ldpart);
     const size_t w_bytes = (size_t)N * Kpad * 2 * HCfg<PREC>::planes, a_bytes = (size_t)M * Kpad * 2 * HCfg<PREC>::planes;
     auto pick_mode = [&](int nNtx, int nMtx, int per_cu) {
         const bool ok = nNtx >= 8 || (nNtx > 0 && 8 % nNtx == 0);
@@ -1209,6 +1375,10 @@
                          int32_t K, const EpiArgs& ep, float* out_f32, int32_t ldo, _Float16* out_h2, int32_t ldh_o,
                          int32_t flags, hipStream_t stream, const float* dotw = nullptr, float* part = nullptr, int32_t ldpart = 0,
                          float* skws = nullptr, size_t skws_bytes = 0);
+int32_t p2w_gemm_chain_h1_impl(int32_t prec, const _Float16* Ah, int32_t ldh_a, const _Float16* W0, float wscale0, int32_t rows, int32_t N0,
+                               int32_t K0, const EpiArgs& ep0, _Float16* e_h, int32_t ldh_e, int32_t flags0, const _Float16* W1, float wscale1,
+                               int32_t N1, const EpiArgs& ep1, float* out_f32, int32_t ldo, _Float16* out_h2, int32_t ldh_o, int32_t flags1,
+                               int* ctl, hipStream_t stream);
 int32_t p2w_sa_conv_h1_impl(int32_t prec, const float* P, int32_t ldp, int32_t n_src, const float* xyzr_src, const int32_t* idx,
                             const int32_t* batch_dst, const float* sf, const int32_t* nbr, const int32_t* deg, int32_t kw,
                             int32_t M, const float* w1r4, const _Float16* W2h, float wscale, int32_t C1, int32_t C2,
diff --git a/pointstowood_amd/engine.py b/pointstowood_amd/engine.py
--- a/pointstowood_amd/engine.py
+++ b/pointstowood_amd/engine.py
@@ -295,6 +295,7 @@
     fp_hoist_ratio: float = 0.5
     range_guard: bool = True
     gemm_stream_k: bool = True
+    res_chain: bool = True
     sa_flags: int = 0
     overlap: bool = True
     search_priority: int = 0
@@ -692,16 +693,26 @@
         if self.gemm_stream_k:
             ws = self._sk_workspace(A.device)
             self._call(name, lib().p2w_gemm_h2_sk, self.prec, ptr(A), ldh_a, ptr(lin.w16), lin.wscale, M, lin.N, lin.K, C.byref(ep),
-                       ptr(out_f32), ldo, ptr(out_h2), ldh_o, ptr(ws), ws.numel(), flags)
+                       ptr(out_f32), ldo, ptr(out_h2), ldh_o, ptr(ws), self._sk_bytes, flags)
             return
         self._call(name, lib().p2w_gemm_h2, self.prec, ptr(A), ldh_a, ptr(lin.w16), lin.wscale, M, lin.N, lin.K, C.byref(ep),
                    ptr(out_f32), ldo, ptr(out_h2), ldh_o, flags)
+
+    def _gemm_h2_chain(self, name, A, ldh_a, M, lin0: Linear, e, ldh_e, lin1: Linear, out_f32=None, ldo=0, out_h2=None, ldh_o=0,
+                       residual=None, ldr=0, residual_h=False, watch0=None, watch1=None):
+        ep0 = self._epilogue(lin0, None, 0, self._watch(watch0, M), None, 0)
+        ep1 = self._epilogue(lin1, residual, ldr, self._watch(watch1, M), None, 0)
+        ws = self._sk_workspace(A.device)
+        self._call(name, lib().p2w_gemm_h2_chain, self.prec, ptr(A), ldh_a, ptr(lin0.w16), lin0.wscale, M, lin0.N, lin0.K, C.byref(ep0),
+                   ptr(e), ldh_e, self.gemm_flags, ptr(lin1.w16), lin1.wscale, lin1.N, C.byref(ep1), ptr(out_f32), ldo, ptr(out_h2), ldh_o,
+                   self.gemm_flags | (GEMM_RESIDUAL_H if residual_h else 0), ptr(ws), ws.numel())
 
     def _sk_workspace(self, dev):
         key = _lib.stream()
         ws = self._sk_ws.get(key)
         if ws is None:
-            ws = self._sk_ws[key] = torch.empty(int(lib().p2w_gemm_h2_sk_ws_bytes()), dtype=torch.uint8, device=dev)
+            self._sk_bytes = int(lib().p2w_gemm_h2_sk_ws_bytes())
+            ws = self._sk_ws[key] = torch.zeros(int(lib().p2w_gemm_h2_chain_ws_bytes()), dtype=torch.uint8, device=dev)
         return ws
 
     def _hoist(self, xh_src, pitch_src, n_src, p, l):
@@ -783,11 +794,13 @@
                 e1, e2 = bufs
                 self._gemm_h2("gemm_res", convh[r0:], pad8(C2), m, p["g1"], out_h2=e1, ldh_o=pad8(E), watch=f"res{l}.1")
                 self._gemm_h2("gemm_res", e1, pad8(E), m, p["g2"], out_h2=e2, ldh_o=pad8(E), watch=f"res{l}.2")
+                last = dict(out_f32=None if out is None else out[r0:], ldo=C2, out_h2=xh[l][r0:], ldh_o=pitch[l],
+                            residual=convh[r0:] if res_h else conv[r0:], ldr=pad8(C2) if res_h else C2, residual_h=res_h)
+                if self.res_chain and self.gemm_stream_k and L.p2w_gemm_h2_chain_rows(prec, m, E, E, C2, self.gemm_flags) > 0:
+                    self._gemm_h2_chain("gemm_res", e2, pad8(E), m, p["g3"], e1, pad8(E), p["g4"], watch0=f"res{l}.3", watch1=f"res{l}.4", **last)
+                    return
                 self._gemm_h2("gemm_res", e2, pad8(E), m, p["g3"], out_h2=e1, ldh_o=pad8(E), watch=f"res{l}.3")
-                self._gemm_h2("gemm_res", e1, pad8(E), m, p["g4"], out_f32=None if out is None else out[r0:], ldo=C2,
-                              out_h2=xh[l][r0:], ldh_o=pitch[l],
-                              residual=convh[r0:] if res_h else conv[r0:], ldr=pad8(C2) if res_h else C2, residual_h=res_h,
-                              watch=f"res{l}.4")
+                self._gemm_h2("gemm_res", e1, pad8(E), m, p["g4"], watch=f"res{l}.4", **last)
             self._chunk_chains(geo, M, E, E // 256, True, lambda rows: (newh(rows, E), newh(rows, E)), res_chunk)
             if l == 3:
                 x3 = out
```

New measurement: 20.71 million, median of 6. About the same (+1.0%).
